# Polochon-street/bliss-rs

Measured on AMD Instinct MI355X. Metric: songs/sec (3-min 22 050 Hz f32) at 1/2/4/8 GPU; HBM GB/s vs roofline, higher is better.
Workload: dtype f32; 1 GPU; configs[1]: batch of 1024 synthetic 3969000-sample (3-min) white-noise f32 PCM buffers per GPU, full 23-feature descriptor set (FeaturesVersion 2); songs_per_gpu=1024, songs_total=1024, features=23, parallelism=single GPU

## Files before the change

bliss-rs_amd/csrc/blissgpu.hip:

```cpp
#include <math.h>
#include <stdio.h>
#include <stdlib.h>
#include <string.h>

#include <algorithm>
#include <atomic>
#include <chrono>
#include <deque>
#include <mutex>
#include <string>
#include <vector>

#include "ctx.hpp"
#include "forest.hpp"

using namespace bg;

namespace {
thread_local std::string g_last_error;

const char* const kKernelNames[K_COUNT] = {
    "fft512_kernel",     "onset_kernel",      "beat_kernel",   "stft8192_kernel", "tune_select_kernel",
    "tune_pass2_kernel", "tune_final_kernel", "chroma_kernel",     "summary_kernel", "assemble_kernel", "pairwise_kernel", "set_distance_kernel", "song_to_song_kernel", "synth_kernel", "rolloff_fix_kernel",
    "dedup_next_kernel", "dedup_walk_kernel", "knn_scan_kernel", "knn_merge_kernel",
    "forest_walk_kernel", "forest_finish_kernel"};
}

namespace bg {
int fail(int code, const char* what, const char* detail) {
    g_last_error = std::string(what) + ": " + (detail ? detail : "");
    return code;
}
}

namespace {

template <typename T>
int upload(T** dst, const std::vector<T>& h) {
    HIP_TRY(hipMalloc((void**)dst, h.size() * sizeof(T)));
    HIP_TRY(hipMemcpy(*dst, h.data(), h.size() * sizeof(T), hipMemcpyHostToDevice));
    return BLISSGPU_OK;
}

int build_tables(blissgpu_ctx* c) {
    const float PI_F = 3.14159265358979323846f;
    std::vector<float2> tw8(8192), tw5(512);
    for (int k = 0; k < 8192; k++) {
        const double a = -2.0 * M_PI * (double)k / 8192.0;
        tw8[k] = make_float2((float)cos(a), (float)sin(a));
    }
    for (int k = 0; k < 512; k++) {
        const double a = -2.0 * M_PI * (double)k / 512.0;
        tw5[k] = make_float2((float)cos(a), (float)sin(a));
    }
    std::vector<float> hann(8192), hannz(512), rwv(BT_LAGLEN), dfwv(BT_WINLEN);
    for (int n = 0; n < 8192; n++) hann[n] = 0.5f * (0.5f - 0.5f * cosf(2.0f * (float)n * PI_F / 8192.0f));
    for (int i = 0; i < 512; i++) hannz[i] = 0.5f * (0.5f * (1.0f - cosf(2.0f * PI_F * (float)i / 512.0f)));
    const float rayparam = 60.0f * (float)SAMPLE_RATE / 120.0f / (float)HOP_B;
    const float dfwvnorm = expf((logf(2.0f) / rayparam) * (float)(BT_WINLEN + 2));
    for (int i = 0; i < BT_LAGLEN; i++) {
        const float i_f = (float)(i + 1);
        rwv[i] = (i_f / (rayparam * rayparam)) * expf(-(i_f * i_f) / (2.0f * (rayparam * rayparam)));
    }
    for (int i = 0; i < BT_WINLEN; i++) dfwv[i] = expf((logf(2.0f) / rayparam) * (float)(i + 1)) / dfwvnorm;
    int rc;
    if ((rc = upload(&c->tw8192, tw8))) return rc;
    if ((rc = upload(&c->tw512, tw5))) return rc;
    if ((rc = upload(&c->hann8192, hann))) return rc;
    if ((rc = upload(&c->hannz512, hannz))) return rc;
    if ((rc = upload(&c->bt_rwv, rwv))) return rc;
    if ((rc = upload(&c->bt_dfwv, dfwv))) return rc;
    const size_t bank_elems = (size_t)(N_TUNING + 1) * BANK_ROWS * BANK_PITCH;
    HIP_TRY(hipMalloc((void**)&c->chroma_bank, bank_elems * sizeof(double)));
    launch_chroma_bank(c->chroma_bank, c->own_stream);
    HIP_TRY(hipGetLastError());
    HIP_TRY(hipStreamSynchronize(c->own_stream));
    c->tables = DeviceTables{c->tw8192, c->tw512, c->hann8192, c->hannz512, c->chroma_bank, c->bt_rwv, c->bt_dfwv};
    return BLISSGPU_OK;
}

std::mutex g_default_mu;
std::vector<int> g_default_devices;
struct DefaultSeat {
    std::mutex mu;
    blissgpu_ctx* ctx = nullptr;
    int fails = 0;
    bool permanent = false;
    std::chrono::steady_clock::time_point retry_at{};
    int rc = BLISSGPU_OK;
    std::string err;
};
std::deque<DefaultSeat> g_default_seats;
std::vector<uint64_t> g_default_batches;
bool g_default_init = false;
std::atomic<int64_t> g_single_song_timeout_ms{600000};

void default_init_locked() {
    if (g_default_init) return;
    g_default_init = true;
    if (const char* e = getenv("BLISSGPU_DEFAULT_DEVICES")) {
        for (const char* p = e; *p;) {
            char* end = nullptr;
            const long v = strtol(p, &end, 10);
            if (end == p) break;
            if (v >= 0 && v < 4096 && g_default_devices.size() < 64) g_default_devices.push_back((int)v);
            p = *end == ',' ? end + 1 : end;
            if (*end && *end != ',') break;
        }
    }
    if (g_default_devices.empty()) {
        int count = 0;
        if (hipGetDeviceCount(&count) != hipSuccess || count < 1) count = 1;
        for (int k = 0; k < count && k < 64; k++) g_default_devices.push_back(k);
    }
    g_default_seats.resize(g_default_devices.size());
    g_default_batches.assign(g_default_devices.size(), 0);
}

}

namespace bg {
int default_ctx_count() {
    std::lock_guard<std::mutex> lk(g_default_mu);
    default_init_locked();
    return (int)g_default_devices.size();
}
int default_ctx_at(int k, blissgpu_ctx** out) {
    DefaultSeat* seat = nullptr;
    int device = 0;
    {
        std::lock_guard<std::mutex> lk(g_default_mu);
        default_init_locked();
        if (k < 0 || k >= (int)g_default_devices.size()) return fail(BLISSGPU_ERR_INVALID, "default context", "no such default device");
        seat = &g_default_seats[(size_t)k];
        device = g_default_devices[(size_t)k];
    }
    std::lock_guard<std::mutex> lk(seat->mu);
    if (!seat->ctx) {
        const auto now = std::chrono::steady_clock::now();
        if (seat->fails == 0 || (!seat->permanent && now >= seat->retry_at)) {
            seat->rc = blissgpu_ctx_create(device, &seat->ctx);
            if (seat->rc) {
                seat->ctx = nullptr;
                seat->fails++;
                seat->permanent = seat->rc == BLISSGPU_ERR_NO_DEVICE || seat->rc == BLISSGPU_ERR_INVALID;
                seat->retry_at = now + std::chrono::milliseconds(std::min(5000, 100 << std::min(seat->fails - 1, 6)));
                seat->err = std::string("default context ") + std::to_string(k) + " (HIP device " + std::to_string(device) + "): " + blissgpu_last_error();
            } else {
                seat->fails = 0;
                seat->permanent = false;
            }
        }
    }
    if (!seat->ctx) return fail(seat->rc, "default context", seat->err.c_str());
    *out = seat->ctx;
    return BLISSGPU_OK;
}
void default_ctx_forget_failures() {
    std::lock_guard<std::mutex> lk(g_default_mu);
    default_init_locked();
    for (DefaultSeat& seat : g_default_seats) {
        std::lock_guard<std::mutex> sl(seat.mu);
        if (!seat.ctx) { seat.fails = 0; seat.permanent = false; seat.rc = BLISSGPU_OK; }
    }
}
namespace {
std::mutex g_live_mu;
std::vector<int> g_live_contexts;
std::mutex g_persistent_mu[64];
}
std::mutex& persistent_kernel_mutex(int device) { return g_persistent_mu[(unsigned)device % 64u]; }
void live_context_add(int device, int delta) {
    std::lock_guard<std::mutex> lk(g_live_mu);
    if (device < 0) return;
    if ((size_t)device >= g_live_contexts.size()) g_live_contexts.resize((size_t)device + 1, 0);
    g_live_contexts[(size_t)device] += delta;
}
int live_contexts(int device) {
    std::lock_guard<std::mutex> lk(g_live_mu);
    return device >= 0 && (size_t)device < g_live_contexts.size() ? g_live_contexts[(size_t)device] : 0;
}
int64_t single_song_timeout_ms() { return g_single_song_timeout_ms.load(); }
int default_ctx(blissgpu_ctx** out) { return default_ctx_at(0, out); }
void default_ctx_count_batch(int k) {
    std::lock_guard<std::mutex> lk(g_default_mu);
    if (k >= 0 && k < (int)g_default_batches.size()) g_default_batches[k]++;
}
}

extern "C" {
int blissgpu_default_device_count(void) { return default_ctx_count(); }
int blissgpu_default_ctx(int k, blissgpu_ctx** ctx) {
    if (!ctx) return fail(BLISSGPU_ERR_INVALID, "blissgpu_default_ctx", "NULL argument");
    *ctx = nullptr;
    return default_ctx_at(k, ctx);
}
int blissgpu_set_single_song_timeout_ms(int64_t ms) {
    constexpr int64_t TEN_YEARS_MS = 10LL * 365 * 24 * 3600 * 1000;
    g_single_song_timeout_ms.store(ms > 0 ? std::min(ms, TEN_YEARS_MS) : 600000);
    return BLISSGPU_OK;
}
int blissgpu_default_reset(void) {
    default_ctx_forget_failures();
    front_revive_all();
    return BLISSGPU_OK;
}
int blissgpu_default_device(int k) {
    std::lock_guard<std::mutex> lk(g_default_mu);
    default_init_locked();
    return (k >= 0 && k < (int)g_default_devices.size()) ? g_default_devices[k] : -1;
}
uint64_t blissgpu_default_device_batches(int k) {
    std::lock_guard<std::mutex> lk(g_default_mu);
    return (k >= 0 && k < (int)g_default_batches.size()) ? g_default_batches[k] : 0;
}
}

namespace {

int is_diag(const float* M, uint32_t d) {
    for (uint32_t i = 0; i < d; i++)
        for (uint32_t j = 0; j < d; j++)
            if (i != j && M[i * d + j] != 0.0f) return 0;
    return 1;
}

}

#define CTX_ENTER(c, who)                                                     \
    if (!(c)) return fail(BLISSGPU_ERR_INVALID, who, "ctx is NULL");          \
    std::lock_guard<std::recursive_mutex> ctx_lock_((c)->mu);                 \
    HIP_TRY(hipSetDevice((c)->device))

extern "C" {

const char* blissgpu_version(void) { return "blissgpu 0.3.0 (gfx950)"; }
const char* blissgpu_last_error(void) { return g_last_error.c_str(); }

const char* blissgpu_strerror(int code) {
    switch (code) {
        case BLISSGPU_OK: return "ok";
        case BLISSGPU_ERR_NO_DEVICE: return "no usable HIP device (this library has no CPU path)";
        case BLISSGPU_ERR_INVALID: return "invalid argument";
        case BLISSGPU_ERR_HIP: return "HIP runtime error";
        case BLISSGPU_ERR_NAN: return "a distance is NaN";
        case BLISSGPU_ERR_OOM: return "out of device memory";
        case BLISSGPU_ERR_RCCL: return "RCCL error";
        case BLISSGPU_ERR_TIMEOUT: return "no default context picked the call up within its deadline";
        default: return "unknown error";
    }
}

uint32_t blissgpu_feature_count(uint32_t v) { return v == BLISSGPU_FEATURES_V1 ? 20u : (v == BLISSGPU_FEATURES_V2 ? 23u : 0u); }

int blissgpu_ctx_create(int device, blissgpu_ctx** out) {
    if (!out) return fail(BLISSGPU_ERR_INVALID, "blissgpu_ctx_create", "ctx is NULL");
    int count = 0;
    hipError_t e = hipGetDeviceCount(&count);
    if (e != hipSuccess || count <= 0 || device < 0 || device >= count)
        return fail(BLISSGPU_ERR_NO_DEVICE, "hipGetDeviceCount", e != hipSuccess ? hipGetErrorString(e) : "no such device");
    HIP_TRY(hipSetDevice(device));
    blissgpu_ctx* c = new blissgpu_ctx();
    c->device = device;
    (void)hipDeviceGetAttribute(&c->n_cus, hipDeviceAttributeMultiprocessorCount, device);
    hipError_t se = hipStreamCreateWithFlags(&c->own_stream, hipStreamNonBlocking);
    if (se != hipSuccess) { delete c; return fail(BLISSGPU_ERR_HIP, "hipStreamCreate", hipGetErrorString(se)); }
    c->stream = c->own_stream;
    int prio_least = 0, prio_greatest = 0;
    (void)hipDeviceGetStreamPriorityRange(&prio_least, &prio_greatest);
    const int prio_aux = prio_greatest;
    se = hipStreamCreateWithPriority(&c->aux_stream, hipStreamNonBlocking, prio_aux);
    if (se == hipSuccess) se = hipStreamCreateWithPriority(&c->chr_stream, hipStreamNonBlocking, prio_greatest);
    if (se == hipSuccess) se = hipEventCreateWithFlags(&c->ev_interop, hipEventDisableTiming);
    if (se == hipSuccess) se = hipHostMalloc((void**)&c->h_scalar, 64, hipHostMallocDefault);
    if (se != hipSuccess) { blissgpu_ctx_destroy(c); return fail(BLISSGPU_ERR_HIP, "aux stream/events", hipGetErrorString(se)); }
    size_t free_b = 0, total_b = 0;
    if (hipMemGetInfo(&free_b, &total_b) == hipSuccess && free_b > 0)
        c->ws_limit = std::max<uint64_t>(256ull << 20, std::min<uint64_t>(64ull << 30, free_b / 3));
    else
        c->ws_limit = 16ull << 30;
    int rc = build_tables(c);
    if (rc) { blissgpu_ctx_destroy(c); return rc; }
    live_context_add(device, 1);
    c->counted_live = true;
    *out = c;
    return BLISSGPU_OK;
}

int blissgpu_ctx_destroy(blissgpu_ctx* c) {
    if (!c) return BLISSGPU_OK;
    if (c->counted_live) live_context_add(c->device, -1);
    {
        std::lock_guard<std::recursive_mutex> lk(c->mu);
        (void)hipSetDevice(c->device);
        (void)hipStreamSynchronize(c->stream);
        if (c->aux_stream) (void)hipStreamSynchronize(c->aux_stream);
        if (c->chr_stream) (void)hipStreamSynchronize(c->chr_stream);
        if (c->mask_stream) { (void)hipStreamSynchronize(c->mask_stream); (void)hipStreamDestroy(c->mask_stream); }
        for (auto& v : c->events)
            for (auto& ev : v) { (void)hipEventDestroy(ev.a); (void)hipEventDestroy(ev.b); }
        (void)hipFree(c->tw8192); (void)hipFree(c->tw512); (void)hipFree(c->hann8192); (void)hipFree(c->hannz512);
        (void)hipFree(c->bt_rwv); (void)hipFree(c->bt_dfwv); (void)hipFree(c->chroma_bank);
        scheduler_release(c);
        c->dbg_tuning.release(); c->dbg_nbpms.release(); c->dbg_chroma.release(); c->dbg_interval.release();
        c->pl_sync.release(); c->pl_keys.release(); c->pl_tmp.release(); c->pl_slots.release(); c->pl_next.release(); c->st_idx.release();
        c->st_a.release(); c->st_b.release(); c->st_m.release(); c->st_dist.release(); c->st_out.release();
        if (c->h_scalar) (void)hipHostFree(c->h_scalar);
        if (c->aux_stream) (void)hipStreamDestroy(c->aux_stream);
        if (c->chr_stream) (void)hipStreamDestroy(c->chr_stream);
        if (c->ev_interop) (void)hipEventDestroy(c->ev_interop);
        if (c->own_stream) (void)hipStreamDestroy(c->own_stream);
    }
    delete c;
    return BLISSGPU_OK;
}

int blissgpu_ctx_set_stream(blissgpu_ctx* c, void* s) {
    CTX_ENTER(c, "blissgpu_ctx_set_stream");
    (void)hipStreamSynchronize(c->stream);
    c->stream = s ? (hipStream_t)s : c->own_stream;
    return BLISSGPU_OK;
}
void* blissgpu_ctx_get_stream(blissgpu_ctx* c) { return c ? (void*)c->stream : nullptr; }

int blissgpu_ctx_wait_stream(blissgpu_ctx* c, void* producer_stream) {
    CTX_ENTER(c, "blissgpu_ctx_wait_stream");
// ... 856 lines not shown
```

bliss-rs_amd/csrc/internal.hpp:

```cpp
#pragma once
#include <hip/hip_runtime.h>
#include <stdint.h>

namespace bg {

constexpr uint32_t SAMPLE_RATE = 22050;
constexpr int W512 = 512;
constexpr int HOP_T = 128;
constexpr int HOP_B = 256;
constexpr int W8192 = 8192;
constexpr int HOP_C = 2205;
constexpr int CBINS = W8192 / 2 + 1;
constexpr int CBINS_PAD = 4128;
constexpr int BANK_PITCH = CBINS_PAD;
constexpr int BANK_ROWS = 12;
constexpr int LOUD_W = 1024;
constexpr int MIN_SAMPLES = 8192;
constexpr int N_TUNING = 100;
constexpr int PIP_LO = 57, PIP_HI = 1483;
constexpr int PIP_MAX_PER_FRAME = 714;
constexpr int CAND_BUDGET_PER_FRAME = 48;
#ifndef COARSE_SHIFT
#define COARSE_SHIFT 17
#endif
constexpr uint32_t COARSE_LOW_MASK = (1u << COARSE_SHIFT) - 1u;
constexpr int H1_BINS = 1 << (31 - COARSE_SHIFT);
constexpr int BT_WINLEN = 512, BT_STEP = 128, BT_LAGLEN = 128;
constexpr int BT_PRE_STRIDE = 264;
constexpr int F512_TILE = 512;
constexpr int CH_TILE = 64;
constexpr int STFT_TILE = 16;

struct SongDesc {
    uint64_t pcm_off;
    uint64_t n;
    uint64_t t_off;
    uint64_t b_off;
    uint64_t c_off;
    uint64_t e_off;
    uint32_t n_t;
    uint32_t n_b;
    uint32_t n_f;
    uint32_t n_c;
    uint32_t n_e;
    uint32_t n_l;
    uint32_t row;
    uint32_t ok;
};

struct RollFix {
    float* mags;
    uint32_t cap;
};
constexpr float ROLLOFF_UNPROVEN = -1.0f;

struct TuningState {
    uint32_t n_peaks;
    uint32_t b_lo, b_hi;
    uint32_t below;
    uint32_t n_cand;
    int32_t tuning_idx;
    uint32_t cand_off;
    uint32_t cand_cap;
};

struct TempoState {
    float tempo;
    uint32_t n_bpms;
};

struct DeviceTables {
    const float2* tw8192;
    const float2* tw512;
    const float* hann8192;
    const float* hannz512;
    const double* chroma_bank;
    const float* bt_rwv;
    const float* bt_dfwv;
};

enum KernelId : int {
    K_FFT512 = 0,
    K_ONSET,
    K_BEAT,
    K_STFT8192,
    K_TUNE_SELECT,
    K_TUNE_PASS2,
    K_TUNE_FINAL,
    K_CHROMA,
    K_SUMMARY,
    K_FINALIZE,
    K_PAIRWISE, K_SET_DISTANCE, K_SONG_TO_SONG,
    K_SYNTH,
    K_ROLLFIX,
    K_DEDUP_NEXT, K_DEDUP_WALK,
    K_KNN_SCAN, K_KNN_MERGE,
    K_FOREST_WALK, K_FOREST_FINISH,
    K_COUNT
};

__device__ __forceinline__ uint32_t find_segment(const uint32_t* __restrict__ prefix, uint32_t n, uint32_t x) {
    uint32_t lo = 0, hi = n;
    while (hi - lo > 1) {
        const uint32_t mid = (lo + hi) >> 1;
        if (prefix[mid] <= x) lo = mid; else hi = mid;
    }
    return lo;
}

struct Workspace {
    float *centroid, *rolloff, *flatness;
    float *flux, *thresholded;
    float* e256;
    uint32_t* zc256;
    float* spec;
    float* frame_max;
    uint32_t* h1;
    uint32_t* hist100;
    TuningState* tuning;
    uint32_t* peak_rec;
    uint32_t* peak_cnt;
    double* cand_mag;
    uint8_t* cand_pb;
    uint32_t* cand_cursor;
    uint32_t cand_cap;
    double* chroma_part;
    double* dbg_chroma;
    double* dbg_interval;
    TempoState* tempo;
    float* run_bpm;
    uint32_t* run_cnt;
    uint32_t runs_pitch;
    float* bt_pre;
    float* summary;
    RollFix* roll_fix;
    size_t roll_fix_bytes;
};

struct Batch {
    const float* pcm;
    const SongDesc* songs;
    uint32_t n_songs;
    const uint32_t* pfx_f;
    const uint32_t* pfx_c;
    const uint32_t* pfx_ct;
    const uint32_t* pfx_cw;
    uint32_t tiles_f, tiles_c, tiles_ct, tiles_cw;
    uint64_t total_b;
    uint32_t max_nb;
    uint32_t max_nt;
};

void launch_fft512(const Batch&, const Workspace&, const DeviceTables&, hipStream_t, bool rolloff_exact_all = false, bool seq_flux = false);
void launch_rolloff_fix(const Batch&, const Workspace&, uint64_t total_t, hipStream_t);
void launch_onset(const Batch&, const Workspace&, hipStream_t);
void launch_beat(const Batch&, const Workspace&, const DeviceTables&, hipStream_t);
void launch_beat_acf(const Batch&, const Workspace&, const DeviceTables&, hipStream_t);
void launch_beat_track(const Batch&, const Workspace&, const DeviceTables&, hipStream_t);
void launch_stft8192(const Batch&, const Workspace&, const DeviceTables&, hipStream_t, int shape = 0);
struct SongRange { uint32_t s0, s1, ct0, ct1, cw0, cw1; };
void launch_tune_select(const Batch&, const Workspace&, hipStream_t, const SongRange* r = nullptr);
void launch_tune_pass2(const Batch&, const Workspace&, hipStream_t, const SongRange* r = nullptr);
void launch_tune_final(const Batch&, const Workspace&, hipStream_t, const SongRange* r = nullptr);
void launch_chroma(const Batch&, const Workspace&, const DeviceTables&, hipStream_t, const SongRange* r = nullptr);
void launch_summary(const Batch&, const Workspace&, hipStream_t);
void launch_finalize(const Batch&, const Workspace&, uint32_t features_version, float* d_out, int32_t* d_status,
                     int32_t* dbg_tuning, uint32_t* dbg_nbpms, hipStream_t);
void launch_chroma_bank(double* bank, hipStream_t);
void launch_pcm_convert(const void* in, int sample_format, uint32_t channels, float* out, uint64_t frames, hipStream_t st);
struct SwrPlan;
hipError_t launch_resample(const void* in, int sample_format, uint32_t channels, uint64_t frames, const SwrPlan& plan,
                           const float* d_bank, float* out, uint64_t n_out, hipStream_t st);
void launch_pair_distance(const float* a, const float* b, uint32_t d, int metric, const float* d_M, float* out, hipStream_t st);
void launch_set_distance(const float* seeds, uint32_t n_seeds, const float* cand, uint64_t n, uint32_t d, int metric,
                         const float* M, float* dist, uint32_t* keys, uint32_t* idx, uint32_t* nan_flag, hipStream_t st);
hipError_t sort_pairs_u32(void* tmp, size_t* tmp_bytes, uint32_t* keys_in, uint32_t* keys_out, uint32_t* vals_in,
                          uint32_t* vals_out, uint32_t n, hipStream_t st, uint32_t* sync = nullptr, uint32_t max_coresident = 0);
void launch_song_to_song(const float* seeds, uint32_t n_seeds, const float* cand, uint32_t n, uint32_t d, int metric,
                         const float* M, uint32_t* order, unsigned long long* slots, uint32_t* sync, uint32_t grid,
                         hipStream_t st);
void launch_dedup_next(const float* x, uint64_t n, uint32_t d, const uint32_t* seq, uint32_t len, const uint32_t* meta,
                       int metric, const float* M, float thr, uint32_t* next, uint32_t* bad, hipStream_t st);
void launch_dedup_walk(const float* x, uint64_t n, uint32_t d, const uint32_t* seq, uint32_t len, const uint32_t* meta,
                       int metric, const float* M, float thr, const uint32_t* next, uint32_t* kept, uint64_t* n_kept,
                       uint32_t* nan_flag, uint32_t* bad, hipStream_t st);
struct KnnPlan {
    uint32_t cap;
    uint32_t qb;
    uint32_t n_split;
    uint32_t blocks_per_split;
    uint32_t grid_qb;
    uint64_t part_keys;
};
KnnPlan knn_plan(uint64_t q, uint64_t n, uint32_t k, int n_cus);
void launch_knn_scan(const float* Q, uint64_t q, const float* X, uint32_t n, uint32_t d, int metric, const float* M,
                     int m_is_diag, const uint32_t* skip, uint32_t k, const KnnPlan& p, unsigned long long* part,
                     uint32_t* nan_flag, uint32_t* bad_flag, hipStream_t st);
void launch_knn_merge(const unsigned long long* part, uint64_t q, uint32_t k, const KnnPlan& p, uint32_t* idx, float* dist,
                      hipStream_t st);
void launch_pairwise(const float* A, uint64_t n, const float* B, uint64_t m, uint32_t d, int metric, const float* M,
                     int m_is_diag, float* out, uint64_t ld_out, hipStream_t);
void launch_synth(float* pcm, const SongDesc* songs, uint32_t n_songs, const uint32_t* pfx_e, uint32_t tiles_e,
                  uint32_t first_song_index, const uint32_t* d_song_index, hipStream_t);

}
```

bliss-rs_amd/csrc/kernels_chroma.hip:

```cpp
#include <float.h>
#include <stdlib.h>

#include <type_traits>

#include "device_utils.hpp"
#include "fft_r16.hpp"
#include "internal.hpp"

namespace bg {

typedef double double4_t __attribute__((ext_vector_type(4)));

__device__ __forceinline__ double tuning_of_slot(int slot) {
    return slot >= N_TUNING ? 0.0 : (-50.0 + (100.0 * 0.01 * (double)slot)) / 100.0;
}

__global__ __launch_bounds__(256) void chroma_bank_kernel(double* __restrict__ bank) {
#pragma clang fp contract(off)
    const int slot = blockIdx.y;
    const int k = blockIdx.x * 256 + threadIdx.x;
    if (k >= BANK_PITCH) return;
    double* out = bank + (size_t)slot * BANK_ROWS * BANK_PITCH;
    if (k >= CBINS) {
        for (int r = 0; r < BANK_ROWS; r++) out[(size_t)r * BANK_PITCH + k] = 0.0;
// ... 291 lines not shown
    f2 v[16];
    if (f_first < sd.n_c) {
        load_frame(f_first, v);
        load_window();
#pragma unroll
        for (int n1 = 0; n1 < 16; n1++) v[n1] = v[n1] * win[n1];
    }
    TRACE_START();
#pragma unroll 1
    for (int fi = 0; fi < STFT_FRAMES_PER_WG; fi++) {
        const uint32_t f = f_first + (uint32_t)(STFT_GROUP * fi);
        if (f >= sd.n_c) break;
        radix16(v);
#pragma unroll
        for (int k1 = 1; k1 < 16; k1++)
            v[R16(k1)] = cmul_pk(v[R16(k1)], tw_at(hi4, k1));
        if constexpr (NARROW) {
            f2 u[16];
#pragma unroll
            for (int k1 = 0; k1 < 16; k1++) ldsf[k1 * EXN1_PITCH + t] = v[R16(k1)].x;
            __syncthreads();
#pragma unroll
            for (int m1 = 0; m1 < 16; m1++) u[m1].x = ldsf[lo4 * EXN1_PITCH + 16 * m1 + hi4];
            __syncthreads();
#pragma unroll
            for (int k1 = 0; k1 < 16; k1++) ldsf[k1 * EXN1_PITCH + t] = v[R16(k1)].y;
            __syncthreads();
#pragma unroll
            for (int m1 = 0; m1 < 16; m1++) u[m1].y = ldsf[lo4 * EXN1_PITCH + 16 * m1 + hi4];
#pragma unroll
            for (int m1 = 0; m1 < 16; m1++) v[m1] = u[m1];
        } else {
#pragma unroll
        for (int k1 = 0; k1 < 16; k1++) lds[k1 * EX1_PITCH + t] = v[R16(k1)];
        TRACE(0);
        __syncthreads();
        TRACE(1);
#pragma unroll
        for (int m1 = 0; m1 < 16; m1++) v[m1] = lds[lo4 * EX1_PITCH + 16 * m1 + hi4];
        }
        radix16(v);
        v[R16(0)] = cmul_pk(v[R16(0)], c_p2);
#pragma unroll
        for (int j1 = 1; j1 < 16; j1++) v[R16(j1)] = cmul_pk(v[R16(j1)], cmul_pk(tw_at(hi4, j1), c_p2));
        TRACE(2);
        __syncthreads();
        TRACE(3);
        if constexpr (NARROW) {
            f2 u[16];
#pragma unroll
            for (int j1 = 0; j1 < 16; j1++) ldsf[j1 * EX2_PITCH + t] = v[R16(j1)].x;
            __syncthreads();
#pragma unroll
            for (int m2 = 0; m2 < 16; m2++) u[m2].x = ldsf[hi4 * EX2_PITCH + 16 * m2 + lo4];
            __syncthreads();
#pragma unroll
            for (int j1 = 0; j1 < 16; j1++) ldsf[j1 * EX2_PITCH + t] = v[R16(j1)].y;
            __syncthreads();
#pragma unroll
            for (int m2 = 0; m2 < 16; m2++) u[m2].y = ldsf[hi4 * EX2_PITCH + 16 * m2 + lo4];
#pragma unroll
            for (int m2 = 0; m2 < 16; m2++) v[m2] = u[m2];
        } else {
#pragma unroll
        for (int j1 = 0; j1 < 16; j1++) lds[j1 * EX2_PITCH + t] = v[R16(j1)];
        TRACE(4);
        __syncthreads();
        TRACE(5);
#pragma unroll
        for (int m2 = 0; m2 < 16; m2++) v[m2] = lds[hi4 * EX2_PITCH + 16 * m2 + lo4];
        }
        radix16(v);
        TRACE(6);
        __syncthreads();
        TRACE(7);
        constexpr int ZOFF = NARROW ? 2048 : 0;
#pragma unroll
        for (int j2 = 8; j2 < 16; j2++) lds[t + 256 * j2 - ZOFF] = v[R16(j2)];
        TRACE(8);
        __syncthreads();
        TRACE(9);
        float m_lo[8], m_hi[8], m_mid = 0.0f;
        float mx = 0.0f;
#pragma unroll
        for (int j = 0; j < 8; j++) {
            const float CJ = CONST_COS32[j], SJ = CONST_SIN32[j];
            const int k = t + 256 * j;
            float sq_k, sq_m;
            const f2 w = j == 0 ? c_sp : cmul_pk_s(c_sp, mk(CJ, -SJ));
            const f2 zm = lds[(k == 0 ? 2048 : 4096 - k) - ZOFF];
            split_pair_sq(v[R16(j)], (j == 0 && t == 0) ? v[R16(0)] : zm, w, sq_k, sq_m);
            m_lo[j] = mag_from_sq(sq_k);
            m_hi[j] = mag_from_sq(sq_m);
            mx = fmaxf(mx, fmaxf(m_lo[j], m_hi[j]));
        }
        if (t == 0) {
            m_mid = mag_from_sq(split_one_sq(v[R16(8)], v[R16(8)], mk(0.0f, -1.0f)));
            mx = fmaxf(mx, m_mid);
        }
        const bool has_next = fi + 1 < STFT_FRAMES_PER_WG && f + STFT_GROUP < sd.n_c;
        if (has_next) load_frame(f + STFT_GROUP, v);
        mx = wave_max_dpp(mx);
        if constexpr (NARROW) __syncthreads();
        float* mags = reinterpret_cast<float*>(lds);
        float* mags_top = mags + MAGS_TOP_W - 4096;
#pragma unroll
        for (int j = 0; j < 8; j++) {
            mags[t + 256 * j] = m_lo[j];
            if (j == 0 && t == 0) mags_top[4096] = m_hi[0];
            else mags[4096 - (t + 256 * j)] = m_hi[j];
        }
        if (t == 0) mags[2048] = m_mid;
        if (t >= 1 && t < CBINS_PAD - 4096) mags_top[4096 + t] = 0.0f;
        {
            int slot = t >> 6;
            asm volatile("" : "+v"(slot));
            if (lane_id() == 0) red[slot] = mx;
        }
        if (t == 0) peak_count = 0;
        TRACE(10);
        __syncthreads();
        TRACE(11);
        auto store_row = [&]() {
            const __amdgpu_buffer_rsrc_t r_row = __builtin_amdgcn_make_buffer_rsrc(
                (void*)(spec + (sd.c_off + f) * (size_t)CBINS_PAD), 0, CBINS_PAD * 4, 0x00020000);
            const u32x4_t* mags4 = reinterpret_cast<const u32x4_t*>(lds);
#pragma unroll
            for (int i = 0; i < 5; i++) {
                const int q = t + 256 * i;
                if (i < 4 || q < CBINS_PAD / 4) {
                    const u32x4_t val = i < 4 ? mags4[q] : mags4[q - 1024 + MAGS_TOP_W / 4];
                    __builtin_amdgcn_raw_buffer_store_b128(val, r_row, 16u * (uint32_t)q, 0, 2);
                }
            }
        };
        store_row();
        mx = fmaxf(fmaxf(red[0], red[1]), fmaxf(red[2], red[3]));
        if (t == 0) frame_max[sd.c_off + f] = mx;
        if (!have_base) {
            if (t == 0) {
                const uint32_t top = coarse_bin((double)mx);
                lhist_base = top > (uint32_t)(LHIST_BINS * 3 / 4) ? top - (uint32_t)(LHIST_BINS * 3 / 4) : 0u;
            }
            have_base = true;
            __syncthreads();
        }
        TRACE(12);
        const uint32_t lbase = lhist_base;
        __builtin_amdgcn_s_setprio(2);
        const double ref = 0.1 * (double)mx;
        const float thr = ref_floor_f32(ref);
        {
            uint32_t hits = 0;
#pragma unroll
            for (int h = 0; h < 2; h++) {
                float sb3[3], se3[3], sa3[3];
#pragma unroll
                for (int q = 0; q < 3; q++) {
                    const int c = t + 256 * (3 * h + q);
                    sb3[q] = mags[c > 0 ? c - 1 : 0];
                    se3[q] = mags[c];
                    sa3[q] = mags[c + 1];
                }
#pragma unroll
                for (int q = 0; q < 3; q++) {
                    const int j = 3 * h + q, c = t + 256 * j;
                    const uint32_t in_range = (256 * j >= PIP_LO && 256 * j + 255 <= PIP_HI) ? 1u : (uint32_t)(c >= PIP_LO) & (uint32_t)(c <= PIP_HI);
                    const uint32_t pk = in_range & (uint32_t)(sa3[q] <= se3[q]) & (uint32_t)(sb3[q] < se3[q]) & (uint32_t)(se3[q] > thr);
                    hits |= pk << j;
                }
            }
            const uint32_t mine = (uint32_t)__popc(hits);
            const uint32_t incl = wave_scan_incl_u32_dpp(mine);
            uint32_t wbase = 0;
            if (lane_id() == 63) wbase = atomicAdd(&peak_count, incl);
            uint32_t pos = (uint32_t)__builtin_amdgcn_readlane((int)wbase, 63) + incl - mine;
#pragma unroll
            for (int j = 0; j < 6; j++)
                if ((hits >> j) & 1u) peak_list[pos++] = (uint16_t)(t + 256 * j);
            TRACE(13);
            __syncthreads();
            TRACE(14);
            const uint32_t n_peaks = peak_count;
            uint32_t* __restrict__ recs = peak_rec + (sd.c_off + f) * (size_t)PIP_MAX_PER_FRAME;
            if (t == 0) peak_cnt[sd.c_off + f] = n_peaks;
            int c_next = t < n_peaks ? (int)peak_list[t] : PIP_LO;
            for (uint32_t i = t; i < n_peaks; i += 256) {
                const int c = c_next;
                const float sb = mags[c - 1], se = mags[c], sa = mags[c + 1];
                c_next = i + 256 < n_peaks ? (int)peak_list[i + 256] : PIP_LO;
                int pb;
                const uint32_t b = peak_classify(sb, se, sa, ref, c, &pb), rel = b - lbase;
                recs[i] = peak_record(b, pb, c);
                if (rel < (uint32_t)LHIST_BINS) atomicAdd(&lhist[rel], 1u);
                else atomicAdd(&hist[b], 1u);
            }
        }
        __builtin_amdgcn_s_setprio(0);
        if (has_next) {
            load_window();
#pragma unroll
            for (int n1 = 0; n1 < 16; n1++) v[n1] = v[n1] * win[n1];
        }
        TRACE(15);
        __syncthreads();
        TRACE(16);
    }
    TRACE_FLUSH();
    if (have_base) {
        const uint32_t lbase = lhist_base;
        for (int i = t; i < LHIST_BINS; i += 256) {
            const uint32_t c = lhist[i];
            if (c) atomicAdd(&hist[lbase + i], c);
        }
    }
}

void launch_stft8192(const Batch& b, const Workspace& w, const DeviceTables& t, hipStream_t st, int shape) {
    if (b.tiles_c == 0) return;
    auto k = stft8192_kernel<false, false>;
    if (shape == 1) k = stft8192_kernel<true, true>;
    else if (shape == 2) k = stft8192_kernel<true, false>;
    else if (shape == 3) k = stft8192_kernel<false, true>;
    hipLaunchKernelGGL(k, dim3((b.tiles_c + 31u) & ~31u), dim3(256), 0, st,
                       b.pcm, b.songs, b.n_songs, b.pfx_c, t.hann8192, t.tw8192, w.spec, w.frame_max, w.h1, w.peak_rec, w.peak_cnt,
                       b.tiles_c);
}

__global__ __launch_bounds__(256) void tune_select_kernel(const SongDesc* __restrict__ songs,
                                                          const uint32_t* __restrict__ h1,
                                                          TuningState* __restrict__ tuning,
                                                          uint32_t* __restrict__ cand_cursor, uint32_t cand_pool,
                                                          uint32_t first_song) {
    __shared__ uint32_t wsum[4];
    __shared__ uint32_t s_total, s_blo, s_bhi;
    const uint32_t s = blockIdx.x + first_song;
    const int tid = threadIdx.x;
    TuningState* ts = tuning + s;
    auto no_peaks = [&]() {
        if (tid == 0) {
            ts->n_peaks = 0; ts->tuning_idx = -1; ts->n_cand = 0; ts->b_lo = 1; ts->b_hi = 0; ts->below = 0;
            ts->cand_off = 0; ts->cand_cap = 0;
        }
    };
    if (!songs[s].ok) { no_peaks(); return; }
    const uint32_t* hist = h1 + (size_t)s * H1_BINS;
    constexpr int PER = H1_BINS / 256;
    uint32_t local[PER], sum = 0;
#pragma unroll
    for (int i = 0; i < PER; i++) { local[i] = hist[tid * PER + i]; sum += local[i]; }
    const uint32_t incl = wave_scan_incl_u32(sum);
    if (lane_id() == 63) wsum[wave_id()] = incl;
    __syncthreads();
    uint32_t base = 0;
    for (int w = 0; w < wave_id(); w++) base += wsum[w];
    if (tid == 255) s_total = base + incl;
    __syncthreads();
    const uint32_t total = s_total;
    uint32_t before = base + incl - sum;
    if (total == 0) { no_peaks(); return; }
    const uint32_t r_lo = (total - 1) / 2, r_hi = total - 1 - r_lo;
    if (tid == 0) { ts->n_peaks = total; ts->n_cand = 0; ts->tuning_idx = -1; }
#pragma unroll
    for (int i = 0; i < PER; i++) {
        const uint32_t c = local[i];
        if (c) {
            if (before <= r_lo && r_lo < before + c) { ts->b_lo = tid * PER + i; ts->below = before; s_blo = tid * PER + i; }
            if (before <= r_hi && r_hi < before + c) { ts->b_hi = tid * PER + i; s_bhi = tid * PER + i; }
        }
        before += c;
    }
    __syncthreads();
    const uint32_t blo = s_blo, bhi = s_bhi;
    uint32_t mine = 0;
#pragma unroll
    for (int i = 0; i < PER; i++) {
        const uint32_t bin = tid * PER + i;
        if (bin >= blo && bin <= bhi) mine += local[i];
    }
    mine = wave_sum(mine);
    if (lane_id() == 0) wsum[wave_id()] = mine;
    __syncthreads();
    if (tid == 0) {
        const uint32_t want = wsum[0] + wsum[1] + wsum[2] + wsum[3];
        const uint32_t off = atomicAdd(cand_cursor, want);
        if (off <= cand_pool && want <= cand_pool - off) {
            ts->cand_off = off;
            ts->cand_cap = want;
        } else {
            atomicSub(cand_cursor, want);
            ts->cand_off = 0;
            ts->cand_cap = 0;
        }
    }
}

void launch_tune_select(const Batch& b, const Workspace& w, hipStream_t st, const SongRange* r) {
    const uint32_t s0 = r ? r->s0 : 0, s1 = r ? r->s1 : b.n_songs;
    if (s1 <= s0) return;
    hipLaunchKernelGGL(tune_select_kernel, dim3(s1 - s0), dim3(256), 0, st, b.songs, w.h1, w.tuning, w.cand_cursor,
                       w.cand_cap, s0);
}

constexpr int P2_SLOW_CAP = 1024;
constexpr int P2_FRAMES_PER_WAVE = CH_TILE / 4;

__global__ __launch_bounds__(256) void tune_pass2_kernel(const SongDesc* __restrict__ songs, uint32_t n_songs,
                                                         const uint32_t* __restrict__ pfx_ct,
                                                         const float* __restrict__ spec,
                                                         const float* __restrict__ frame_max,
                                                         const uint32_t* __restrict__ peak_rec,
                                                         const uint32_t* __restrict__ peak_cnt,
                                                         TuningState* __restrict__ tuning,
                                                         uint32_t* __restrict__ hist100,
                                                         double* __restrict__ cand_mag,
                                                         uint8_t* __restrict__ cand_pb, uint32_t first_tile) {
    __shared__ uint32_t hist[N_TUNING];
    __shared__ uint32_t slow_list[4][P2_SLOW_CAP];
    const uint32_t bx = blockIdx.x + first_tile;
    const uint32_t s = find_segment(pfx_ct, n_songs, bx);
    const SongDesc sd = songs[s];
    const uint32_t tile = bx - pfx_ct[s];
    const int tid = threadIdx.x, lane = lane_id(), wave = wave_id();
    TuningState* ts = tuning + s;
    const uint32_t b_lo = ts->b_lo, b_hi = ts->b_hi;
    if (ts->n_peaks == 0) return;
    const uint32_t cand_off = ts->cand_off;
    const uint32_t cand_cap = ts->cand_cap;
    const bool pooled = cand_cap != 0;
    if (tid < N_TUNING) hist[tid] = 0;
    __syncthreads();
    uint32_t n_slow = 0;

    auto flush = [&]() {
        for (uint32_t i = lane; i < n_slow; i += WAVE) {
            const uint32_t e = slow_list[wave][i];
            const int c = (int)(e & 0xFFFFu);
            const uint32_t f = tile * CH_TILE + wave + 4 * (e >> 16);
            const float* row = spec + (sd.c_off + f) * (size_t)CBINS_PAD;
            const double ref = 0.1 * (double)frame_max[sd.c_off + f];
            double mag, pitch;
            if (pip_peak_core(row[c - 1], row[c], row[c + 1], ref, c, &mag, &pitch)) {
                const uint32_t b = coarse_bin(mag);
                if (b > b_hi) {
                    atomicAdd(&hist[pitch_bin(pitch)], 1u);
                } else if (b >= b_lo) {
                    const uint32_t slot = atomicAdd(&ts->n_cand, 1u);
                    if (pooled && slot < cand_cap) {
                        cand_mag[cand_off + slot] = mag;
                        cand_pb[cand_off + slot] = (uint8_t)pitch_bin(pitch);
                    }
                }
            }
        }
        __builtin_amdgcn_wave_barrier();
        n_slow = 0;
    };
    uint32_t n_rec_next = 0;
    {
        const uint32_t f0 = tile * CH_TILE + wave;
        if (f0 < sd.n_c) n_rec_next = peak_cnt[sd.c_off + f0];
    }
    for (int i = 0; i < P2_FRAMES_PER_WAVE; i++) {
        const uint32_t f = tile * CH_TILE + wave + 4 * i;
        if (f >= sd.n_c) break;
        const uint32_t n_rec = n_rec_next < (uint32_t)PIP_MAX_PER_FRAME ? n_rec_next : (uint32_t)PIP_MAX_PER_FRAME;
        if (i + 1 < P2_FRAMES_PER_WAVE && f + 4 < sd.n_c) n_rec_next = peak_cnt[sd.c_off + f + 4];
        const uint32_t* __restrict__ recs = peak_rec + (sd.c_off + f) * (size_t)PIP_MAX_PER_FRAME;
        if (n_slow + PIP_MAX_PER_FRAME > P2_SLOW_CAP) flush();
        for (uint32_t j0 = 0; j0 < n_rec; j0 += 4 * WAVE) {
            uint32_t r4[4];
#pragma unroll
            for (int u = 0; u < 4; u++) {
                const uint32_t j = j0 + WAVE * u + lane;
                r4[u] = j < n_rec ? recs[j] : 0xFFFFFFFFu;
            }
#pragma unroll
            for (int u = 0; u < 4; u++) {
                if (j0 + WAVE * u >= n_rec) break;
                const uint32_t j = j0 + WAVE * u + lane;
                bool slow = false;
                uint32_t c = 0;
                if (j < n_rec) {
                    const uint32_t r = r4[u];
                    const uint32_t b = r >> 18, pbf = (r >> 11) & 0x7Fu;
                    c = r & 0x7FFu;
                    if (b > b_hi) {
                        if (pbf) atomicAdd(&hist[pbf - 1], 1u);
                        else slow = true;
                    } else if (b >= b_lo) {
                        slow = true;
                    }
                }
                const uint64_t mask = __ballot(slow);
                if (mask) {
                    if (slow) slow_list[wave][n_slow + (uint32_t)__popcll(mask & ((1ull << lane) - 1ull))] = ((uint32_t)i << 16) | c;
                    n_slow += (uint32_t)__popcll(mask);
                }
            }
        }
    }
    __builtin_amdgcn_wave_barrier();
    flush();
    __syncthreads();
    if (tid < N_TUNING && hist[tid]) atomicAdd(&hist100[(size_t)s * N_TUNING + tid], hist[tid]);
}

void launch_tune_pass2(const Batch& b, const Workspace& w, hipStream_t st, const SongRange* r) {
    const uint32_t t0 = r ? r->ct0 : 0, t1 = r ? r->ct1 : b.tiles_ct;
    if (t1 <= t0) return;
    hipLaunchKernelGGL(tune_pass2_kernel, dim3(t1 - t0), dim3(256), 0, st, b.songs, b.n_songs, b.pfx_ct, w.spec,
                       w.frame_max, w.peak_rec, w.peak_cnt, w.tuning, w.hist100, w.cand_mag, w.cand_pb, t0);
}

template <typename ForEach>
__device__ uint64_t block_radix_select(ForEach&& for_each, uint32_t rank, uint32_t* hist, uint32_t* s_digit, uint32_t* s_rank,
                                       uint32_t* s_wave) {
    const int tid = threadIdx.x;
    uint64_t prefix = 0, mask = 0;
    for (int shift = 56; shift >= 0; shift -= 8) {
        hist[tid] = 0;
        __syncthreads();
        for_each([&](double mag, int) {
            const uint64_t k = f64_key(mag);
            const bool in = (k & mask) == prefix;
            const uint32_t d = (uint32_t)(k >> shift) & 0xFFu;
            const uint64_t m = __ballot(in);
            if (m != 0) {
                const int first = __ffsll((unsigned long long)m) - 1;
                const uint32_t d0 = (uint32_t)__shfl((int)d, first, WAVE);
                if (__ballot(in && d == d0) == m) {
                    if (lane_id() == first) atomicAdd(&hist[d0], (uint32_t)__popcll(m));
                } else if (in) {
                    atomicAdd(&hist[d], 1u);
                }
            }
        });
        __syncthreads();
        {
            const uint32_t h = hist[tid];
            const uint32_t incl = wave_scan_incl_u32(h);
            if (lane_id() == 63) s_wave[wave_id()] = incl;
            __syncthreads();
            uint32_t below = incl - h;
            for (int w = 0; w < wave_id(); w++) below += s_wave[w];
            if (h != 0 && below <= rank && rank < below + h) {
                *s_digit = (uint32_t)tid;
                *s_rank = rank - below;
            }
        }
        __syncthreads();
        prefix |= (uint64_t)(*s_digit) << shift;
        mask |= 0xFFull << shift;
        rank = *s_rank;
        __syncthreads();
    }
    return prefix;
}

__global__ __launch_bounds__(256) void tune_final_kernel(const SongDesc* __restrict__ songs,
                                                         TuningState* __restrict__ tuning,
                                                         const uint32_t* __restrict__ hist100,
                                                         const double* __restrict__ cand_mag,
                                                         const uint8_t* __restrict__ cand_pb,
                                                         const float* __restrict__ spec,
                                                         const float* __restrict__ frame_max,
                                                         const uint32_t* __restrict__ peak_rec,
                                                         const uint32_t* __restrict__ peak_cnt, uint32_t first_song) {
    __shared__ uint32_t hist[256];
    __shared__ uint32_t s_digit, s_rank, s_cnt_le, s_wave[4];
    __shared__ unsigned long long s_min_gt;
    const uint32_t s = blockIdx.x + first_song;
    const int tid = threadIdx.x;
    TuningState* ts = tuning + s;
    const SongDesc sd = songs[s];
    if (!sd.ok || ts->n_peaks == 0) return;
    const uint32_t total = ts->n_peaks, nc = ts->n_cand;
    const uint32_t r_lo = (total - 1) / 2, r_hi = total - 1 - r_lo;
    const uint32_t k_lo = r_lo - ts->below, k_hi = r_hi - ts->below;
    const uint32_t b_lo = ts->b_lo, b_hi = ts->b_hi;
    const bool pooled = ts->cand_cap != 0 && nc == ts->cand_cap;
    const double* v = cand_mag + ts->cand_off;
    const uint8_t* pb = cand_pb + ts->cand_off;

    auto for_each = [&](auto&& fn) {
        if (pooled) {
            for (uint32_t i0 = tid; i0 < nc; i0 += 8 * 256) {
                double m8[8];
                int b8[8];
#pragma unroll
                for (int u = 0; u < 8; u++) {
                    const uint32_t i = i0 + 256u * u;
                    m8[u] = i < nc ? v[i] : 0.0;
                    b8[u] = i < nc ? (int)pb[i] : 0;
                }
#pragma unroll
                for (int u = 0; u < 8; u++)
                    if (i0 + 256u * u < nc) fn(m8[u], b8[u]);
            }
        } else {
            for (uint32_t f = 0; f < sd.n_c; f++) {
                const uint32_t n_rec_raw = peak_cnt[sd.c_off + f];
                const uint32_t n_rec = n_rec_raw < (uint32_t)PIP_MAX_PER_FRAME ? n_rec_raw : (uint32_t)PIP_MAX_PER_FRAME;
                const uint32_t* __restrict__ recs = peak_rec + (sd.c_off + f) * (size_t)PIP_MAX_PER_FRAME;
                const float* __restrict__ row = spec + (sd.c_off + f) * (size_t)CBINS_PAD;
                const double ref = 0.1 * (double)frame_max[sd.c_off + f];
                for (uint32_t j = tid; j < n_rec; j += 256) {
                    const uint32_t r = recs[j], b = r >> 18;
                    if (b < b_lo || b > b_hi) continue;
                    const int c = (int)(r & 0x7FFu);
                    double mag, pitch;
                    if (pip_peak_core(row[c - 1], row[c], row[c + 1], ref, c, &mag, &pitch)) fn(mag, pitch_bin(pitch));
                }
            }
        }
    };

    const uint64_t key_lo = block_radix_select(for_each, k_lo, hist, &s_digit, &s_rank, s_wave);
    uint64_t key_hi = key_lo;
    if (k_hi != k_lo) {
        if (tid == 0) { s_cnt_le = 0; s_min_gt = ~0ull; }
        __syncthreads();
        uint32_t cnt = 0;
        unsigned long long mn = ~0ull;
        for_each([&](double mag, int) {
            const uint64_t k = f64_key(mag);
            if (k <= key_lo) cnt++;
            else if (k < mn) mn = k;
        });
        atomicAdd(&s_cnt_le, cnt);
        atomicMin(&s_min_gt, mn);
        __syncthreads();
        if (s_cnt_le <= k_hi) key_hi = s_min_gt;
    }
    double thr;
    {
#pragma clang fp contract(off)
        const double lo = key_f64(key_lo), hi = key_f64(key_hi);
        thr = lo + (hi - lo) / 2.0;
    }
    __syncthreads();
    if (tid < N_TUNING) hist[tid] = hist100[(size_t)s * N_TUNING + tid];
    __syncthreads();
    for_each([&](double mag, int bin) {
        if (mag >= thr) atomicAdd(&hist[bin], 1u);
    });
    __syncthreads();
    if (tid == 0) {
        uint32_t best = 0;
        for (uint32_t k = 1; k < N_TUNING; k++)
            if (hist[k] > hist[best]) best = k;
        ts->tuning_idx = (int32_t)best;
    }
}

void launch_tune_final(const Batch& b, const Workspace& w, hipStream_t st, const SongRange* r) {
    const uint32_t s0 = r ? r->s0 : 0, s1 = r ? r->s1 : b.n_songs;
    if (s1 <= s0) return;
    hipLaunchKernelGGL(tune_final_kernel, dim3(s1 - s0), dim3(256), 0, st, b.songs, w.tuning, w.hist100,
                       w.cand_mag, w.cand_pb, w.spec, w.frame_max, w.peak_rec, w.peak_cnt, s0);
}

static constexpr int TMPL_LEN[10] = {2, 2, 2, 2, 2, 2, 3, 3, 3, 3};
static constexpr int TMPL_PC[10][3] = {{0, 1, 0}, {0, 2, 0}, {0, 3, 0}, {0, 4, 0}, {0, 5, 0},
                                       {0, 6, 0}, {0, 4, 7}, {0, 3, 7}, {0, 3, 6}, {0, 4, 8}};

template <int T>
__device__ __forceinline__ double interval_feature(const double (&c)[12]) {
    double acc = 0.0;
#pragma unroll
    for (int shift = 0; shift < 12; shift++) {
        const int r0 = (TMPL_PC[T][0] + shift) % 12, r1 = (TMPL_PC[T][1] + shift) % 12;
        if (TMPL_LEN[T] == 2) {
            acc += c[r0 < r1 ? r0 : r1] * c[r0 < r1 ? r1 : r0];
        } else {
            const int r2 = (TMPL_PC[T][2] + shift) % 12;
            const int lo = r0 < r1 ? (r0 < r2 ? r0 : r2) : (r1 < r2 ? r1 : r2);
            const int hi = r0 > r1 ? (r0 > r2 ? r0 : r2) : (r1 > r2 ? r1 : r2);
            const int mid = r0 + r1 + r2 - lo - hi;
            acc += (c[lo] * c[mid]) * c[hi];
        }
    }
    return acc;
}

__global__ __launch_bounds__(256) void chroma_kernel(const SongDesc* __restrict__ songs, uint32_t n_songs, const uint32_t* __restrict__ pfx_cw,
                              const uint32_t* __restrict__ pfx_ct, const float* __restrict__ spec,
                              const double* __restrict__ bank, const TuningState* __restrict__ tuning,
                              double* __restrict__ chroma_part, double* __restrict__ dbg_chroma, uint32_t first_wg);

void launch_chroma(const Batch& b, const Workspace& w, const DeviceTables& t, hipStream_t st, const SongRange* r) {
    const uint32_t g0 = r ? r->cw0 : 0, g1 = r ? r->cw1 : b.tiles_cw;
    if (g1 <= g0) return;
    hipLaunchKernelGGL(chroma_kernel, dim3(g1 - g0), dim3(256), 0, st, b.songs, b.n_songs, b.pfx_cw, b.pfx_ct, w.spec,
                       t.chroma_bank, w.tuning, w.chroma_part, w.dbg_chroma, g0);
}

#ifndef BG_PROBE_REPLACES_CHROMA_KERNEL
__global__ __launch_bounds__(256) void chroma_kernel(const SongDesc* __restrict__ songs, uint32_t n_songs,
                                                     const uint32_t* __restrict__ pfx_cw,
                                                     const uint32_t* __restrict__ pfx_ct,
                                                     const float* __restrict__ spec,
                                                     const double* __restrict__ bank,
                                                     const TuningState* __restrict__ tuning,
                                                     double* __restrict__ chroma_part,
                                                     double* __restrict__ dbg_chroma, uint32_t first_wg) {
    __shared__ double tile_c[4][4][16][13];
    const uint32_t bx = blockIdx.x + first_wg;
    const uint32_t s = find_segment(pfx_cw, n_songs, bx);
    const SongDesc sd = songs[s];
    const int lane = lane_id(), wave = wave_id();
    const uint32_t tile64 = (bx - pfx_cw[s]) * 4 + wave;
    const uint32_t n_tiles = pfx_ct[s + 1] - pfx_ct[s];
    if (tile64 >= n_tiles) return;
    const int i16 = lane & 15, g = lane >> 4;
    const int tidx = tuning[s].tuning_idx;
    const int slot = (tidx < 0) ? N_TUNING : tidx;
    const uint32_t f0 = tile64 * CH_TILE;

    const double* __restrict__ arow = bank + ((size_t)slot * BANK_ROWS + (i16 < BANK_ROWS ? i16 : BANK_ROWS - 1)) * BANK_PITCH + 8 * g;
    const float* brow[4];
#pragma unroll
    for (int q = 0; q < 4; q++) {
        uint32_t fj = f0 + 16 * q + i16;
        if (fj >= sd.n_c) fj = sd.n_c - 1;
        brow[q] = spec + (sd.c_off + fj) * (size_t)CBINS_PAD + 8 * g;
    }
    double4_t acc[4][2];
#pragma unroll
    for (int q = 0; q < 4; q++) { acc[q][0] = double4_t{0.0, 0.0, 0.0, 0.0}; acc[q][1] = double4_t{0.0, 0.0, 0.0, 0.0}; }
    struct KBlock {
        double4_t a[2];
        float4 b[2][4];
    };
    auto k_load = [&](int k0, KBlock& kb) {
#pragma unroll
        for (int u = 0; u < 2; u++) kb.a[u] = *reinterpret_cast<const double4_t*>(arow + k0 + 4 * u);
#pragma unroll
        for (int q = 0; q < 4; q++)
#pragma unroll
            for (int u = 0; u < 2; u++) kb.b[u][q] = *reinterpret_cast<const float4*>(brow[q] + k0 + 4 * u);
        __builtin_amdgcn_sched_barrier(0);
    };
    auto k_mma = [&](const KBlock& kb) {
#pragma unroll
        for (int u = 0; u < 2; u++) {
#pragma unroll
            for (int q = 0; q < 4; q++) {
                const float4 v = kb.b[u][q];
                const double b0 = (double)v.x * (double)v.x, b1 = (double)v.y * (double)v.y;
                const double b2 = (double)v.z * (double)v.z, b3 = (double)v.w * (double)v.w;
                acc[q][0] = __builtin_amdgcn_mfma_f64_16x16x4f64(kb.a[u].x, b0, acc[q][0], 0, 0, 0);
                acc[q][1] = __builtin_amdgcn_mfma_f64_16x16x4f64(kb.a[u].y, b1, acc[q][1], 0, 0, 0);
                acc[q][0] = __builtin_amdgcn_mfma_f64_16x16x4f64(kb.a[u].z, b2, acc[q][0], 0, 0, 0);
                acc[q][1] = __builtin_amdgcn_mfma_f64_16x16x4f64(kb.a[u].w, b3, acc[q][1], 0, 0, 0);
            }
        }
    };
    constexpr int KBLOCKS = CBINS_PAD / 32;
    static_assert(CBINS_PAD % 32 == 0 && BANK_PITCH == CBINS_PAD && KBLOCKS % 2 == 1, "pairs of blocks and one last block");
    KBlock k0buf, k1buf;
    k_load(0, k0buf);
#pragma unroll 1
    for (int kb = 0; kb + 2 < KBLOCKS; kb += 2) {
        k_load(32 * (kb + 1), k1buf);
        k_mma(k0buf);
        k_load(32 * (kb + 2), k0buf);
        k_mma(k1buf);
    }
    k_mma(k0buf);
#pragma unroll
    for (int q = 0; q < 4; q++) {
        const double4_t cacc = acc[q][0] + acc[q][1];
#pragma unroll
        for (int r = 0; r < 3; r++) tile_c[wave][q][i16][g + 4 * r] = cacc[r];
    }
    __builtin_amdgcn_wave_barrier();
    double feat[10];
#pragma unroll
    for (int t = 0; t < 10; t++) feat[t] = 0.0;
    if (f0 + lane < sd.n_c) {
        double c[12], sum = 0.0;
#pragma unroll
        for (int k = 0; k < 12; k++) { c[k] = tile_c[wave][lane >> 4][lane & 15][k]; sum += fabs(c[k]); }
        if (sum < DBL_MIN) sum = 1.0;
        if (dbg_chroma) {
#pragma unroll
            for (int k = 0; k < 12; k++) dbg_chroma[(sd.c_off + f0 + lane) * 12 + k] = c[k] / sum;
        }
        double esum = 0.0;
#pragma unroll
        for (int k = 0; k < 12; k++) { c[k] = exp((c[k] / sum) * 15.0); esum += fabs(c[k]); }
        if (esum < 0.0001) esum = 1.0;
#pragma unroll
        for (int k = 0; k < 12; k++) c[k] /= esum;
        feat[0] = interval_feature<0>(c); feat[1] = interval_feature<1>(c);
        feat[2] = interval_feature<2>(c); feat[3] = interval_feature<3>(c);
        feat[4] = interval_feature<4>(c); feat[5] = interval_feature<5>(c);
        feat[6] = interval_feature<6>(c); feat[7] = interval_feature<7>(c);
        feat[8] = interval_feature<8>(c); feat[9] = interval_feature<9>(c);
    }
#pragma unroll
    for (int t = 0; t < 10; t++) {
        double v = feat[t];
        const double v1 = __shfl(v, (lane & 15) + 16, WAVE), v2 = __shfl(v, (lane & 15) + 32, WAVE), v3 = __shfl(v, (lane & 15) + 48, WAVE);
        v = __shfl(v, lane & 15, WAVE);
        v = ((v + v1) + v2) + v3;
#pragma unroll
        for (int off = 8; off > 0; off >>= 1) v += __shfl_xor(v, off, WAVE);
        if (lane == 0) chroma_part[(size_t)(pfx_ct[s] + tile64) * 10 + t] = v;
    }
}

#endif

}
```

bliss-rs_amd/csrc/kernels_fft512.hip:

```cpp
#include <float.h>
#include <stdlib.h>

#include <type_traits>

#include "device_utils.hpp"
#include "fft_r16.hpp"
#include "internal.hpp"

namespace bg {

#ifndef FFT512_PAIR_SPLIT
#define FFT512_PAIR_SPLIT 1
#endif
constexpr int GROUPS_PER_WG = 16;
constexpr int FRAMES_PER_GROUP = F512_TILE / GROUPS_PER_WG;
constexpr float ROLL_GUARD = 704.0f / 16777216.0f;
constexpr int GRP_PITCH = 272;

typedef unsigned int u32x2_t __attribute__((ext_vector_type(2)));
__device__ __forceinline__ f2 buf_load_f2(__amdgpu_buffer_rsrc_t r, uint32_t voff, uint32_t soff) {
    const u32x2_t v = __builtin_amdgcn_raw_buffer_load_b64(r, voff, soff, 0);
    return mk(__uint_as_float(v.x), __uint_as_float(v.y));
}

template <int CTRL>
__device__ __forceinline__ float dpp_mov(float v) {
    return __int_as_float(__builtin_amdgcn_update_dpp(0, __float_as_int(v), CTRL, 0xF, 0xF, true));
}
template <int CTRL>
__device__ __forceinline__ int dpp_mov(int v) {
    return __builtin_amdgcn_update_dpp(0, v, CTRL, 0xF, 0xF, true);
}
constexpr int DPP_QUAD_XOR1 = 0xB1, DPP_QUAD_XOR2 = 0x4E, DPP_ROW_HALF_MIRROR = 0x141, DPP_ROW_MIRROR = 0x140;
template <typename T>
__device__ __forceinline__ T row16_sum(T v) {
    v += dpp_mov<DPP_QUAD_XOR1>(v);
    v += dpp_mov<DPP_QUAD_XOR2>(v);
    v += dpp_mov<DPP_ROW_HALF_MIRROR>(v);
    v += dpp_mov<DPP_ROW_MIRROR>(v);
    return v;
}
__device__ __forceinline__ double row16_prod(double v) {
    auto step = [](double x, auto ctrl) {
        const long long b = __double_as_longlong(x);
        const int lo = dpp_mov<decltype(ctrl)::value>((int)(b & 0xFFFFFFFFll)), hi = dpp_mov<decltype(ctrl)::value>((int)(b >> 32));
        return x * __longlong_as_double(((long long)hi << 32) | (unsigned int)lo);
    };
    v = step(v, std::integral_constant<int, DPP_QUAD_XOR1>{});
    v = step(v, std::integral_constant<int, DPP_QUAD_XOR2>{});
    v = step(v, std::integral_constant<int, DPP_ROW_HALF_MIRROR>{});
    v = step(v, std::integral_constant<int, DPP_ROW_MIRROR>{});
    return v;
}
__device__ __forceinline__ float row16_scan_incl(float v) {
    v += dpp_mov<0x111>(v);
    v += dpp_mov<0x112>(v);
    v += dpp_mov<0x114>(v);
    v += dpp_mov<0x118>(v);
    return v;
}

#define BG_DPP_STEP(OP, DST, SRC, CTRL) OP " " DST ", " SRC ", " SRC " " CTRL " row_mask:0xf bank_mask:0xf bound_ctrl:1\n\t"
__device__ __forceinline__ void row16_sum3_scan1(float in_a, float in_b, float in_c, float in_d, float& a, float& b, float& c, float& d) {
    asm("s_nop 1\n\t"
        BG_DPP_STEP("v_add_f32_dpp", "%0", "%4", "quad_perm:[1,0,3,2]") BG_DPP_STEP("v_add_f32_dpp", "%1", "%5", "quad_perm:[1,0,3,2]")
        BG_DPP_STEP("v_add_f32_dpp", "%2", "%6", "row_shr:1") BG_DPP_STEP("v_add_f32_dpp", "%3", "%7", "quad_perm:[1,0,3,2]")
        BG_DPP_STEP("v_add_f32_dpp", "%0", "%0", "quad_perm:[2,3,0,1]") BG_DPP_STEP("v_add_f32_dpp", "%1", "%1", "quad_perm:[2,3,0,1]")
        BG_DPP_STEP("v_add_f32_dpp", "%2", "%2", "row_shr:2") BG_DPP_STEP("v_add_f32_dpp", "%3", "%3", "quad_perm:[2,3,0,1]")
        BG_DPP_STEP("v_add_f32_dpp", "%0", "%0", "row_half_mirror") BG_DPP_STEP("v_add_f32_dpp", "%1", "%1", "row_half_mirror")
        BG_DPP_STEP("v_add_f32_dpp", "%2", "%2", "row_shr:4") BG_DPP_STEP("v_add_f32_dpp", "%3", "%3", "row_half_mirror")
        BG_DPP_STEP("v_add_f32_dpp", "%0", "%0", "row_mirror") BG_DPP_STEP("v_add_f32_dpp", "%1", "%1", "row_mirror")
        BG_DPP_STEP("v_add_f32_dpp", "%2", "%2", "row_shr:8") BG_DPP_STEP("v_add_f32_dpp", "%3", "%3", "row_mirror")
        : "=&v"(a), "=&v"(b), "=&v"(c), "=&v"(d)
        : "v"(in_a), "v"(in_b), "v"(in_c), "v"(in_d));
}
#define BG_DPP3(CTRL)                                                                                           \
    BG_DPP_STEP("v_add_f32_dpp", "%0", "%0", CTRL) BG_DPP_STEP("v_add_f32_dpp", "%1", "%1", CTRL) BG_DPP_STEP("v_add_u32_dpp", "%2", "%2", CTRL)
__device__ __forceinline__ void row16_sum2f_1u(float& a, float& b, uint32_t& c) {
    asm("s_nop 1\n\t" BG_DPP3("quad_perm:[1,0,3,2]") BG_DPP3("quad_perm:[2,3,0,1]") BG_DPP3("row_half_mirror") BG_DPP3("row_mirror")
        : "+v"(a), "+v"(b), "+v"(c));
}

struct FrameMags {
    float m[16];
    float nyq;
};

template <int R>
__device__ __forceinline__ f2& row(f2 (&raw)[16], int n1) { return raw[(R + n1) & 15]; }

__device__ __forceinline__ void fft512_load(__amdgpu_buffer_rsrc_t r_x, long rel_start, int l, f2 (&raw)[16]) {
    if (rel_start >= 0) {
        const uint32_t xoff = (uint32_t)((rel_start + 2 * l) * 4);
#pragma unroll
        for (int n1 = 0; n1 < 16; n1++) raw[n1] = buf_load_f2(r_x, xoff, 128u * n1);
    } else {
#pragma unroll
        for (int n1 = 0; n1 < 16; n1++) {
            const long idx = rel_start + 32 * n1 + 2 * l;
            raw[n1] = mk(0.0f, 0.0f);
            if (idx >= 0) raw[n1] = buf_load_f2(r_x, (uint32_t)(idx * 4), 0);
        }
    }
}

struct RegTables {
    f2 win[16];
    f2 tw256[16];
    f2 tw512[16];
};

template <int R>
__device__ __forceinline__ void fft512_compute(f2 (&raw)[16], int l, f2* tile, const RegTables& tabs, FrameMags& out) {
    f2 v[16];
    __builtin_amdgcn_s_setprio(0);
#pragma unroll
    for (int n1 = 0; n1 < 16; n1++) v[n1] = row<R>(raw, n1) * tabs.win[n1];
    radix16(v);
#pragma unroll
    for (int k1 = 1; k1 < 16; k1++) v[R16(k1)] = cmul_pk(v[R16(k1)], tabs.tw256[k1]);
    __builtin_amdgcn_s_setprio(2);
#pragma unroll
    for (int k1 = 0; k1 < 16; k1++) tile[k1 * 17 + l] = v[R16(k1)];
    __builtin_amdgcn_wave_barrier();
#pragma unroll
    for (int n2 = 0; n2 < 16; n2++) v[n2] = tile[l * 17 + n2];
    __builtin_amdgcn_wave_barrier();
    __builtin_amdgcn_s_setprio(0);
    radix16(v);
    __builtin_amdgcn_s_setprio(2);
#pragma unroll
    for (int k2 = 0; k2 < 16; k2++) tile[k2 * 17 + l] = v[R16(k2)];
    __builtin_amdgcn_wave_barrier();
    const f2 z0 = tile[0];
#if FFT512_PAIR_SPLIT
    {
        const f2 zk = tile[l * 17], zm = tile[(l == 0) ? 0 : 17 * (16 - l)];
        out.m[0] = mag_from_sq(split_one_sq(zk, zm, tabs.tw512[0]));
    }
    float mir[8];
#pragma unroll
    for (int e = 1; e <= 8; e++) {
        const f2 zk = tile[l * 17 + e], zm = tile[17 * (15 - l) + 16 - e];
        float sq_k, sq_m;
        split_pair_sq(zk, zm, tabs.tw512[e], sq_k, sq_m);
        out.m[e] = mag_from_sq(sq_k);
        if (e < 8) mir[e] = mag_from_sq(sq_m);
    }
#pragma unroll
    for (int e = 9; e < 16; e++) out.m[e] = dpp_mov<DPP_ROW_MIRROR>(mir[16 - e]);
#else
#pragma unroll
    for (int e = 0; e < 16; e++) {
        const f2 zk = tile[l * 17 + e];
        const int mi = (e == 0) ? ((l == 0) ? 0 : 17 * (16 - l)) : (17 * (15 - l) + 16 - e);
        const f2 zm = tile[mi];
        out.m[e] = mag_from_sq(split_one_sq(zk, zm, tabs.tw512[e]));
    }
#endif
    if (l == 0) out.m[0] = 2.0f * fabsf(z0.x + z0.y);
    out.nyq = 2.0f * fabsf(z0.x - z0.y);
    __builtin_amdgcn_wave_barrier();
}

__device__ __forceinline__ void add_lane_bit(uint32_t& acc, uint64_t mask) {
    asm("v_addc_co_u32_e64 %0, vcc, 0, %0, %1" : "+v"(acc) : "s"(mask) : "vcc");
}

__device__ __forceinline__ void stats128(const f2 r0, const f2 r1, const f2 r2, const f2 r3, const f2 before, bool song_start,
                                         float& ss, uint32_t& zc) {
    ss += ((r0.x * r0.x + r0.y * r0.y) + (r1.x * r1.x + r1.y * r1.y)) + ((r2.x * r2.x + r2.y * r2.y) + (r3.x * r3.x + r3.y * r3.y));
    constexpr uint64_t LOW = 0x0001000100010001ull;
    const uint64_t x0 = __ballot(r0.x > 0.0f), y0 = __ballot(r0.y > 0.0f), x1 = __ballot(r1.x > 0.0f), y1 = __ballot(r1.y > 0.0f);
    const uint64_t x2 = __ballot(r2.x > 0.0f), y2 = __ballot(r2.y > 0.0f), x3 = __ballot(r3.x > 0.0f), y3 = __ballot(r3.y > 0.0f);
    const uint64_t yb = __ballot(before.y > 0.0f), start = __builtin_amdgcn_ballot_w64(song_start);
    auto shifted = [&](uint64_t y, uint64_t prev_bits) { return ((y << 1) & ~LOW) | prev_bits; };
    const uint64_t p0 = (((yb >> 15) & ~start) | (x0 & start)) & LOW;
    add_lane_bit(zc, x0 ^ y0);
    add_lane_bit(zc, x0 ^ shifted(y0, p0));
    add_lane_bit(zc, x1 ^ y1);
    add_lane_bit(zc, x1 ^ shifted(y1, (y0 >> 15) & LOW));
    add_lane_bit(zc, x2 ^ y2);
    add_lane_bit(zc, x2 ^ shifted(y2, (y1 >> 15) & LOW));
    add_lane_bit(zc, x3 ^ y3);
    add_lane_bit(zc, x3 ^ shifted(y3, (y2 >> 15) & LOW));
}

template <bool ROLLOFF_EXACT_ALL, bool SEQ_FLUX>
__global__ __launch_bounds__(256, 2) void fft512_kernel(const float* __restrict__ pcm,
                                                        const SongDesc* __restrict__ songs, uint32_t n_songs,
                                                        const uint32_t* __restrict__ pfx_f,
                                                        const float* __restrict__ hannz,
                                                        const float2* __restrict__ tw512,
                                                        float* __restrict__ centroid, float* __restrict__ rolloff,
                                                        float* __restrict__ flatness, float* __restrict__ flux,
                                                        float* __restrict__ e256, uint32_t* __restrict__ zc256,
                                                        const RollFix* __restrict__ fix) {
    __shared__ f2 lds[GROUPS_PER_WG * GRP_PITCH];
    __shared__ float halo[GROUPS_PER_WG][16 * 16 + 1];
    RegTables tabs;
    {
        const int l0 = threadIdx.x & 15;
#pragma unroll
        for (int i = 0; i < 16; i++) {
            const float2 a = tw512[2 * ((i * l0) & 255)], b = tw512[16 * l0 + i];
            tabs.win[i] = mk(hannz[2 * (16 * i + l0)], hannz[2 * (16 * i + l0) + 1]);
            tabs.tw256[i] = mk(a.x, a.y);
            tabs.tw512[i] = mk(b.x, b.y);
        }
    }
    const uint32_t s = find_segment(pfx_f, n_songs, blockIdx.x);
    const SongDesc sd = songs[s];
    const uint32_t tile_idx = blockIdx.x - pfx_f[s];
    const int grp = threadIdx.x >> 4, l = threadIdx.x & 15;
    f2* tile = lds + grp * GRP_PITCH;

    const long k_begin = (long)tile_idx * F512_TILE + (long)grp * FRAMES_PER_GROUP;
    const long k_end = (k_begin + FRAMES_PER_GROUP < (long)sd.n_f) ? k_begin + FRAMES_PER_GROUP : (long)sd.n_f;

    const long tile_first = (long)tile_idx * F512_TILE * HOP_T - (W512 - HOP_T) - HOP_T;
    const long base = tile_first > 0 ? tile_first : 0;
    const uint64_t avail = (sd.n - (uint64_t)base) * 4;
    const __amdgpu_buffer_rsrc_t r_x = __builtin_amdgcn_make_buffer_rsrc(
        (void*)(pcm + sd.pcm_off + base), 0, (uint32_t)(avail < 0xFFFFFFFFull ? avail : 0xFFFFFFFFull), 0x00020000);

    FrameMags A, B;
    const bool active = k_begin < (long)sd.n_f;
    const int len = active ? (int)(k_end - k_begin) : 0;
    const long left_t = (long)sd.n_t - k_begin, left_b = (long)sd.n_b - (k_begin >> 1);
    const int lim_t = left_t < 0 ? 0 : (left_t > FRAMES_PER_GROUP ? FRAMES_PER_GROUP : (int)left_t);
    const int lim_b = left_b < 0 ? 0 : (left_b > FRAMES_PER_GROUP ? FRAMES_PER_GROUP : (int)left_b);
    const bool at_song_start = k_begin == 0;
    const uint32_t xoff0 = (uint32_t)(((k_begin + 2) * HOP_T - HOP_T - base + 2 * l) * 4);
    f2 raw[16];
    const bool share = active && grp > 0;
    if (active && k_begin >= 1 && !share) {
        fft512_load(r_x, k_begin * HOP_T - W512 - base, l, raw);
        fft512_compute<0>(raw, l, tile, tabs, A);
    } else {
#pragma unroll
        for (int e = 0; e < 16; e++) A.m[e] = 0.0f;
        A.nyq = 0.0f;
    }
    if (active) fft512_load(r_x, (k_begin + 1) * HOP_T - W512 - base, l, raw);

    float ss_acc = 0.0f;
    uint32_t zc_acc = 0;
    float st_total = 0.0f, st_wtotal = 0.0f, st_mant = 1.0f;
    int st_ints = 0;
    const float freq_per_bin = (float)SAMPLE_RATE / (float)W512;

    auto frame = [&](auto jc, int r_lane, FrameMags& cur, FrameMags& prev) {
        constexpr int J = decltype(jc)::value;
        const int r = __builtin_amdgcn_readfirstlane(r_lane);
        constexpr int R = (4 * J) & 15;
        stats128(row<R>(raw, 12), row<R>(raw, 13), row<R>(raw, 14), row<R>(raw, 15), row<R>(raw, 11), at_song_start && r == 0, ss_acc, zc_acc);
        __builtin_amdgcn_sched_barrier(0);
        fft512_compute<R>(raw, l, tile, tabs, cur);
        if (r + 1 < len) {
            const uint32_t soff = (uint32_t)r * (uint32_t)(HOP_T * 4);
#pragma unroll
            for (int n1 = 0; n1 < 4; n1++) row<R>(raw, n1) = buf_load_f2(r_x, xoff0, soff + 128u * n1);
        }
        if (J & 1) {
            float ss = ss_acc;
            uint32_t zc = zc_acc;
            const int qr = (r - 1) >> 1;
            const long q = (k_begin >> 1) + qr;
            ss_acc = 0.0f;
            zc_acc = 0;
            float f = 0.0f;
            if constexpr (SEQ_FLUX) {
#pragma unroll 1
            for (int step = 0; step < 16; step++) {
                const float carry = dpp_mov<0x111>(f);
                if (l == step) {
                    f = carry;
#pragma unroll
                    for (int e = 0; e < 16; e++) f += fmaxf(cur.m[e] - prev.m[e], 0.0f);
                }
            }
            f = __shfl(f, (threadIdx.x & 48) + 15, 64) + fmaxf(cur.nyq - prev.nyq, 0.0f);
            ss = row16_sum(ss);
            zc = (uint32_t)row16_sum((int)zc);
            } else {
#pragma unroll
            for (int i = 0; i < 8; i++) {
                const f2 d = mk(cur.m[2 * i], cur.m[2 * i + 1]) - mk(prev.m[2 * i], prev.m[2 * i + 1]);
                f += fmaxf(d.x, 0.0f);
                f += fmaxf(d.y, 0.0f);
            }
            if (l == 0) f += fmaxf(cur.nyq - prev.nyq, 0.0f);
            row16_sum2f_1u(ss, f, zc);
            }
            if (l == 0) { e256[sd.e_off + q] = ss; zc256[sd.e_off + q] = zc; }
            if (J == 1 && share && r == 1) {
#pragma unroll
                for (int e = 0; e < 16; e++) halo[grp][16 * e + l] = cur.m[e];
                if (l == 0) halo[grp][256] = cur.nyq;
            } else if (l == 0 && qr < lim_b) {
                flux[sd.b_off + q] = f;
            }
        }
        if (r < lim_t) {
            const float m15 = (l == 15) ? cur.nyq : cur.m[15];
            f2 s2 = mk(0.0f, 0.0f), e2 = mk(0.0f, 0.0f), q2 = mk(0.0f, 0.0f);
#pragma unroll
            for (int i = 0; i < 8; i++) {
                const f2 mp = mk(cur.m[2 * i], i == 7 ? m15 : cur.m[2 * i + 1]);
                s2 = s2 + mp;
                e2 = e2 + mp * mk((float)(2 * i), (float)(2 * i + 1));
                q2 = q2 + mp * mp;
            }
            auto hadd = [](f2 v) __attribute__((always_inline)) { float r; asm("v_add_f32 %0, %1, %2" : "=v"(r) : "v"(v.x), "v"(v.y)); return r; };
            const float sum = hadd(s2), sqsum = hadd(q2);
            const float wsum = (float)(16 * l) * sum + hadd(e2);
            float total, wtotal, incl, cum_total;
            row16_sum3_scan1(sum, wsum, sqsum, sqsum, total, wtotal, incl, cum_total);
            const float thr = cum_total * 0.95f;
            float d = (incl - sqsum) - thr;
            float near;
            uint32_t signs = 0;
#pragma unroll
            for (int i = 0; i < 8; i++) {
                const float m0 = cur.m[2 * i], m1 = i == 7 ? m15 : cur.m[2 * i + 1];
                const float d0 = fmaf(m0, m0, d);
                d = fmaf(m1, m1, d0);
                signs = __builtin_amdgcn_alignbit(signs, __float_as_uint(d0), 31);
                signs = __builtin_amdgcn_alignbit(signs, __float_as_uint(d), 31);
                if (i == 0) asm("v_min_f32 %0, |%1|, |%2|" : "=v"(near) : "v"(d0), "v"(d));
                else asm("v_min3_f32 %0, %0, |%1|, |%2|" : "+v"(near) : "v"(d0), "v"(d));
            }
            const bool risky = ROLLOFF_EXACT_ALL || (cum_total != 0.0f && (!(near > cum_total * ROLL_GUARD) || cum_total < 1e-30f));
            int expo = 0, zero = 0;
            double mant = 1.0;
#pragma unroll
            for (int h = 0; h < 2; h++) {
                const float c7 = h == 1 ? m15 : cur.m[7];
                const float* c8 = cur.m + 8 * h;
                double g = ((double)c8[0] * (double)c8[1]) * ((double)c8[2] * (double)c8[3]);
                g *= 3.273390607896142e150;
                g *= ((double)c8[4] * (double)c8[5]) * ((double)c8[6] * (double)c7);
                if (g == 0.0) zero = 1;
                const uint64_t bits = (uint64_t)__double_as_longlong(g);
                expo += (int)(bits >> 52);
                mant *= __longlong_as_double((long long)((bits & 0xFFFFFFFFFFFFFull) | 0x3FF0000000000000ull));
            }
            const int red = row16_sum((int)((uint32_t)__popc(signs) | ((uint32_t)zero << 9) | ((uint32_t)expo << 14)));
            const int c = red & 511, any_zero = (red >> 9) & 31, exps = (int)((uint32_t)red >> 14);
            mant = row16_prod(mant);
            const bool mine = l == (r & 15);
            const uint64_t risky_lanes = __builtin_amdgcn_ballot_w64(risky);
            const uint32_t grp_mask = (uint32_t)(risky_lanes >> (threadIdx.x & 48)) & 0xFFFFu;
            const int packed = c | (any_zero ? 1 << 9 : 0) | (cum_total == 0.0f ? 1 << 10 : 0) | (exps << 11) | (grp_mask != 0 ? 1 << 27 : 0);
            st_total = mine ? total : st_total;
            st_wtotal = mine ? wtotal : st_wtotal;
            st_ints = mine ? packed : st_ints;
            st_mant = mine ? (float)mant : st_mant;
            if (risky_lanes != 0) {
                if (grp_mask != 0) {
                    float4* dst = reinterpret_cast<float4*>(fix->mags + (size_t)(sd.t_off + (uint64_t)(k_begin + r)) * 256 + 16 * l);
                    dst[0] = make_float4(cur.m[0], cur.m[1], cur.m[2], cur.m[3]);
                    dst[1] = make_float4(cur.m[4], cur.m[5], cur.m[6], cur.m[7]);
                    dst[2] = make_float4(cur.m[8], cur.m[9], cur.m[10], cur.m[11]);
                    dst[3] = make_float4(cur.m[12], cur.m[13], cur.m[14], m15);
                }
            }
        }
    };
    auto finish16 = [&](int r16) {
        const int r = r16 + l;
        const long k = k_begin + r;
        if (r < len && r < lim_t) {
            const float cbin = (st_total == 0.0f) ? 0.0f : st_wtotal / st_total;
            const int st_c = st_ints & 511, st_exps = (st_ints >> 11) & 0xFFFF;
            const float rbin = (st_ints & (1 << 10)) ? 0.0f : (float)((st_c < 256) ? st_c + 1 : 256);
            float flat = 0.0f;
            if (!(st_ints & (1 << 9))) {
                const float geo = exp2f((log2f(st_mant) + (float)st_exps) / 256.0f - (1023.0f + 500.0f) / 8.0f);
                if (geo != 0.0f) flat = geo / (st_total / 256.0f);
            }
            centroid[sd.t_off + k] = freq_per_bin * fmaxf(cbin, 0.0f);
            rolloff[sd.t_off + k] = (st_ints & (1 << 27)) ? ROLLOFF_UNPROVEN : freq_per_bin * fmaxf(rbin, 0.0f);
            flatness[sd.t_off + k] = flat;
        }
    };

    for (int rb = 0; rb < len; rb += 4) {
        frame(std::integral_constant<int, 0>{}, rb, B, A);
        __builtin_amdgcn_sched_barrier(0);
        if (rb + 1 < len) frame(std::integral_constant<int, 1>{}, rb + 1, B, A);
        __builtin_amdgcn_sched_barrier(0);
        if (rb + 2 < len) frame(std::integral_constant<int, 2>{}, rb + 2, A, B);
        __builtin_amdgcn_sched_barrier(0);
        if (rb + 3 < len) frame(std::integral_constant<int, 3>{}, rb + 3, A, B);
        __builtin_amdgcn_sched_barrier(0);
        if ((rb & 15) == 12 || rb + 4 >= len) finish16(rb & ~15);
    }

    __syncthreads();
    if (grp + 1 < GROUPS_PER_WG && k_begin + FRAMES_PER_GROUP + 1 < (long)sd.n_f) {
        const long q = (k_begin + FRAMES_PER_GROUP) >> 1;
        float f = 0.0f;
        const float cn = halo[grp + 1][256];
        if constexpr (SEQ_FLUX) {
        float hc[16];
#pragma unroll
        for (int e = 0; e < 16; e++) hc[e] = halo[grp + 1][16 * e + l];
#pragma unroll 1
        for (int step = 0; step < 16; step++) {
            const float carry = dpp_mov<0x111>(f);
            if (l == step) {
                f = carry;
#pragma unroll
                for (int e = 0; e < 16; e++) f += fmaxf(hc[e] - A.m[e], 0.0f);
            }
        }
        f = __shfl(f, (threadIdx.x & 48) + 15, 64) + fmaxf(cn - A.nyq, 0.0f);
        } else {
#pragma unroll
        for (int e = 0; e < 16; e++) {
            const float c = halo[grp + 1][16 * e + l];
            f += fmaxf(c - A.m[e], 0.0f);
        }
        if (l == 0) f += fmaxf(cn - A.nyq, 0.0f);
        f = row16_sum(f);
        }
        if (l == 0 && q < (long)sd.n_b) flux[sd.b_off + q] = f;
    }

    if (active && k_end == (long)sd.n_f) {
        const float* __restrict__ x = pcm + sd.pcm_off;
        const uint64_t t0 = (uint64_t)sd.n_f * HOP_T;
        for (uint64_t q = t0 >> 8; q < (uint64_t)sd.n_e; q++) {
            const uint64_t lo = (q << 8) > t0 ? (q << 8) : t0;
            const uint64_t hi = ((q + 1) << 8) < sd.n ? ((q + 1) << 8) : sd.n;
            for (uint64_t i = lo + (uint64_t)l; i < hi; i += 16) {
                const float v = x[i], pv = x[i - 1];
                ss_acc += v * v;
                zc_acc += ((v > 0.0f) != (pv > 0.0f)) ? 1u : 0u;
            }
            const float ss = row16_sum(ss_acc);
            const uint32_t zc = (uint32_t)row16_sum((int)zc_acc);
            if (l == 0) { e256[sd.e_off + q] = ss; zc256[sd.e_off + q] = zc; }
            ss_acc = 0.0f;
            zc_acc = 0;
        }
    }
}

void launch_fft512(const Batch& b, const Workspace& w, const DeviceTables& t, hipStream_t st, bool rolloff_exact_all, bool seq_flux) {
    if (b.tiles_f == 0) return;
    auto k = fft512_kernel<false, false>;
    if (rolloff_exact_all && seq_flux) k = fft512_kernel<true, true>;
    else if (rolloff_exact_all) k = fft512_kernel<true, false>;
    else if (seq_flux) k = fft512_kernel<false, true>;
    hipLaunchKernelGGL(k, dim3(b.tiles_f), dim3(256), 0, st, b.pcm, b.songs, b.n_songs, b.pfx_f, t.hannz512,
                       t.tw512, w.centroid, w.rolloff, w.flatness, w.flux, w.e256, w.zc256, w.roll_fix);
}

}
```

bliss-rs_amd/csrc/scheduler.hip:

```cpp
#include <string.h>

#include <algorithm>
#include <chrono>
#include <condition_variable>
#include <numeric>

#include "coalescing_front.hpp"
#include "ctx.hpp"

using namespace bg;

namespace {

inline size_t align_up(size_t x, size_t a) { return (x + a - 1) / a * a; }

void fill_counts(SongDesc& d) {
    const uint64_t n = d.n;
    d.n_t = (uint32_t)((n - W512) / HOP_T + 1);
    d.n_b = (uint32_t)((n - W512) / HOP_B + 1);
    d.n_f = std::max(d.n_t, 2u * d.n_b);
    d.n_c = (uint32_t)ceilf((float)n / (float)HOP_C);
    d.n_e = (uint32_t)((n + 255) / 256);
    d.n_l = (uint32_t)((n + LOUD_W - 1) / LOUD_W);
}

size_t song_ws_bytes(const SongDesc& d) {
    if (!d.ok) return 256;
    size_t b = 0;
    b += (size_t)d.n_t * 12 + (size_t)d.n_b * 8 + (size_t)d.n_e * 8;
    b += (size_t)d.n_c * (CBINS_PAD * 4 + 4);
    b += (size_t)H1_BINS * 4 + N_TUNING * 4 + sizeof(TuningState) + sizeof(TempoState);
    b += (size_t)d.n_c * CAND_BUDGET_PER_FRAME * 9;
    b += (size_t)d.n_c * (PIP_MAX_PER_FRAME * 4 + 4);
    b += ((size_t)d.n_c / CH_TILE + 1) * 80;
    b += ((size_t)d.n_b / BT_STEP + 2) * (8 + BT_PRE_STRIDE * 4);
    return b + 4096;
}

struct Carver {
    uint8_t* base;
    size_t off = 0;
    template <typename T>
    T* take(size_t n) {
        off = align_up(off, 256);
        T* p = reinterpret_cast<T*>(base + off);
        off += n * sizeof(T);
        return p;
    }
};

struct ChunkTotals {
    uint64_t tot_t = 0, tot_b = 0, tot_c = 0, tot_e = 0;
    uint32_t max_nb = 0, max_nt = 0, max_runs = 1;
    uint32_t tiles_ct = 0;
    uint64_t cand_cap = 0;
};

Workspace carve(uint8_t* base, uint32_t ns, const ChunkTotals& t, size_t* bytes) {
    Carver m{base};
    Workspace w{};
    w.centroid = m.take<float>(t.tot_t); w.rolloff = m.take<float>(t.tot_t); w.flatness = m.take<float>(t.tot_t);
    w.flux = m.take<float>(t.tot_b); w.thresholded = m.take<float>(t.tot_b);
    w.e256 = m.take<float>(t.tot_e); w.zc256 = m.take<uint32_t>(t.tot_e);
    static_assert((size_t)(CBINS_PAD + PIP_MAX_PER_FRAME) * 4 * HOP_T >= (size_t)256 * 4 * HOP_C,
                  "the borrowed stretch must hold one 256-word entry per timbral frame: bytes per chroma frame x samples per "
                  "timbral frame >= bytes per entry x samples per chroma frame");
    w.spec = m.take<float>(t.tot_c * CBINS_PAD + 64);
    w.peak_rec = m.take<uint32_t>(t.tot_c * PIP_MAX_PER_FRAME);
    w.roll_fix_bytes = (size_t)(reinterpret_cast<uint8_t*>(w.peak_rec + t.tot_c * PIP_MAX_PER_FRAME) - reinterpret_cast<uint8_t*>(w.spec));
    w.frame_max = m.take<float>(t.tot_c);
    w.roll_fix = m.take<RollFix>(1);
    w.h1 = m.take<uint32_t>((size_t)ns * H1_BINS); w.hist100 = m.take<uint32_t>((size_t)ns * N_TUNING);
    w.tuning = m.take<TuningState>(ns);
    w.peak_cnt = m.take<uint32_t>(t.tot_c);
    w.cand_mag = m.take<double>(t.cand_cap); w.cand_pb = m.take<uint8_t>(t.cand_cap);
    w.cand_cursor = m.take<uint32_t>(4);
    w.cand_cap = (uint32_t)t.cand_cap;
    w.chroma_part = m.take<double>((size_t)t.tiles_ct * 10 + 16);
    w.tempo = m.take<TempoState>(ns);
    w.run_bpm = m.take<float>((size_t)ns * t.max_runs); w.run_cnt = m.take<uint32_t>((size_t)ns * t.max_runs);
    w.runs_pitch = t.max_runs;
    w.bt_pre = m.take<float>((size_t)(t.tot_b / BT_STEP + ns + 1) * BT_PRE_STRIDE);
    w.summary = m.take<float>((size_t)ns * 16);
    *bytes = m.off + 4096;
    return w;
}

int ensure_mask_stream(blissgpu_ctx* c, int cus) {
    cus = std::max(1, std::min(cus, c->n_cus));
    if (c->mask_stream && c->mask_cus == cus) return BLISSGPU_OK;
    if (c->mask_stream) { (void)hipStreamSynchronize(c->mask_stream); (void)hipStreamDestroy(c->mask_stream); c->mask_stream = nullptr; }
    std::vector<uint32_t> mask((size_t)(c->n_cus + 31) / 32, 0u);
    for (int i = 0; i < cus; i++) mask[(size_t)i / 32] |= 1u << (i % 32);
    HIP_TRY(hipExtStreamCreateWithCUMask(&c->mask_stream, (uint32_t)mask.size(), mask.data()));
    c->mask_cus = cus;
    return BLISSGPU_OK;
}

int ensure_slot_events(ChunkSlot& s) {
    if (s.ev_free) return BLISSGPU_OK;
    hipEvent_t* evs[] = {&s.ev_start, &s.ev_fork, &s.ev_stft, &s.ev_sel, &s.ev_tune, &s.ev_sum, &s.ev_chroma, &s.ev_desc, &s.ev_free, &s.ev_acf, &s.ev_beat};
    for (hipEvent_t* e : evs) HIP_TRY(hipEventCreateWithFlags(e, hipEventDisableTiming));
    for (hipEvent_t& e : s.ev_piece) HIP_TRY(hipEventCreateWithFlags(&e, hipEventDisableTiming));
    return BLISSGPU_OK;
}

int chunk_front(blissgpu_ctx* c, ChunkSlot& slot, const float* d_pcm, SongDesc* songs, uint32_t ns, bool only_chunk) {
    int rc = ensure_slot_events(slot);
    if (rc) return rc;
    std::vector<uint32_t> pfx_f(ns + 1, 0), pfx_c(ns + 1, 0), pfx_ct(ns + 1, 0), pfx_cw(ns + 1, 0);
    ChunkTotals t;
    for (uint32_t i = 0; i < ns; i++) {
        SongDesc& d = songs[i];
        d.t_off = t.tot_t; d.b_off = t.tot_b; d.c_off = t.tot_c; d.e_off = t.tot_e;
        if (d.ok) {
            t.tot_t += d.n_t; t.tot_b += d.n_b; t.tot_c += d.n_c; t.tot_e += d.n_e;
            t.max_nb = std::max(t.max_nb, d.n_b);
            t.max_nt = std::max(t.max_nt, d.n_t);
            t.max_runs = std::max(t.max_runs, d.n_b / BT_STEP + 1);
        }
        pfx_f[i + 1] = pfx_f[i] + (d.ok ? (d.n_f + F512_TILE - 1) / F512_TILE : 0);
        pfx_c[i + 1] = pfx_c[i] + (d.ok ? 4 * ((d.n_c + 4 * STFT_TILE - 1) / (4 * STFT_TILE)) : 0);
        pfx_ct[i + 1] = pfx_ct[i] + (d.ok ? (d.n_c + CH_TILE - 1) / CH_TILE : 0);
        pfx_cw[i + 1] = pfx_cw[i] + (d.ok ? (d.n_c + 4 * CH_TILE - 1) / (4 * CH_TILE) : 0);
    }
    t.tiles_ct = pfx_ct[ns];
    t.cand_cap = std::min<uint64_t>(t.tot_c * (uint64_t)c->cand_budget, 0xFFFFFF00ull) + 64;

    const size_t desc_bytes = align_up(ns * sizeof(SongDesc), 256) + 4 * align_up((ns + 1) * 4, 256) + 256;
    size_t need = 0;
    (void)carve(nullptr, ns, t, &need);
    if ((rc = slot.desc.ensure(desc_bytes))) return rc;
    if ((rc = slot.slab.ensure(need))) return rc;
    if (slot.used) HIP_TRY(hipEventSynchronize(slot.ev_desc));
    if ((rc = slot.h_desc.ensure(desc_bytes))) return rc;

    hipStream_t st = c->stream, sb = c->serial ? c->stream : c->aux_stream, sc = c->serial ? c->stream : c->chr_stream;
    const bool multi = !c->serial;
    if (slot.used && multi) HIP_TRY(hipStreamWaitEvent(st, slot.ev_free, 0));

    uint8_t* h = slot.h_desc.p;
    size_t o = 0;
    const size_t o_songs = o; memcpy(h + o, songs, ns * sizeof(SongDesc)); o = align_up(o + ns * sizeof(SongDesc), 256);
    const size_t o_f = o; memcpy(h + o, pfx_f.data(), (ns + 1) * 4); o = align_up(o + (ns + 1) * 4, 256);
    const size_t o_c = o; memcpy(h + o, pfx_c.data(), (ns + 1) * 4); o = align_up(o + (ns + 1) * 4, 256);
    const size_t o_ct = o; memcpy(h + o, pfx_ct.data(), (ns + 1) * 4); o = align_up(o + (ns + 1) * 4, 256);
    const size_t o_cw = o; memcpy(h + o, pfx_cw.data(), (ns + 1) * 4); o = align_up(o + (ns + 1) * 4, 256);
    HIP_TRY(hipMemcpyAsync(slot.desc.p, h, o, hipMemcpyHostToDevice, st));
    slot.used = true;

    Batch& b = slot.batch;
    b = Batch{};
    b.pcm = d_pcm;
    b.songs = reinterpret_cast<const SongDesc*>(slot.desc.p + o_songs);
    b.n_songs = ns;
    b.pfx_f = reinterpret_cast<const uint32_t*>(slot.desc.p + o_f);
    b.pfx_c = reinterpret_cast<const uint32_t*>(slot.desc.p + o_c);
    b.pfx_ct = reinterpret_cast<const uint32_t*>(slot.desc.p + o_ct);
    b.pfx_cw = reinterpret_cast<const uint32_t*>(slot.desc.p + o_cw);
    b.tiles_f = pfx_f[ns]; b.tiles_c = pfx_c[ns]; b.tiles_ct = pfx_ct[ns]; b.tiles_cw = pfx_cw[ns];
    b.total_b = t.tot_b; b.max_nb = t.max_nb; b.max_nt = t.max_nt;

    size_t used_bytes = 0;
    slot.ws = carve(slot.slab.p, ns, t, &used_bytes);
    slot.ws.dbg_chroma = nullptr;
    slot.ws.dbg_interval = nullptr;
    if (c->debug_chroma) {
        if ((rc = c->dbg_chroma.ensure((size_t)t.tot_c * 12 + 12))) return rc;
        if ((rc = c->dbg_interval.ensure((size_t)ns * 10))) return rc;
        slot.ws.dbg_chroma = c->dbg_chroma.p;
        slot.ws.dbg_interval = c->dbg_interval.p;
    }
    const Workspace& w = slot.ws;
    c->last_ws = w;
    c->last_songs.assign(songs, songs + ns);
    {
        RollFix rf{};
        if ((uint64_t)w.roll_fix_bytes / (256 * 4) < t.tot_t)
            return fail(BLISSGPU_ERR_INVALID, "chunk_front", "internal: the borrowed stretch cannot hold one exact-rolloff entry per timbral frame");
        rf.cap = (uint32_t)t.tot_t;
        rf.mags = w.spec;
        memcpy(h + o, &rf, sizeof(rf));
        HIP_TRY(hipMemcpyAsync(w.roll_fix, h + o, sizeof(rf), hipMemcpyHostToDevice, st));
    }
    HIP_TRY(hipEventRecord(slot.ev_desc, st));

    HIP_TRY(hipMemsetAsync(w.h1, 0, (size_t)ns * H1_BINS * 4, st));
    HIP_TRY(hipMemsetAsync(w.hist100, 0, (size_t)ns * N_TUNING * 4, st));
    HIP_TRY(hipMemsetAsync(w.cand_cursor, 0, 16, st));
    { Prof p(c, K_FFT512); launch_fft512(b, w, c->tables, st, c->rolloff_exact_all, c->flux_order); }
    { Prof p(c, K_ROLLFIX); launch_rolloff_fix(b, w, t.tot_t, st); }
    if (multi) {
        HIP_TRY(hipEventRecord(slot.ev_fork, st));
        HIP_TRY(hipStreamWaitEvent(sb, slot.ev_fork, 0));
    }
    { Prof p(c, K_ONSET, sb); launch_onset(b, w, sb); }
    { Prof p(c, K_SUMMARY, sb); launch_summary(b, w, sb); }
    slot.beat_masked = multi && c->tail_mode >= 2;
    if (slot.beat_masked) {
        if ((rc = ensure_mask_stream(c, c->tail_mode))) return rc;
        { Prof p(c, K_BEAT, sb); launch_beat_acf(b, w, c->tables, sb); }
        HIP_TRY(hipEventRecord(slot.ev_acf, sb));
        HIP_TRY(hipStreamWaitEvent(c->mask_stream, slot.ev_acf, 0));
        { Prof p(c, K_BEAT, c->mask_stream); launch_beat_track(b, w, c->tables, c->mask_stream); }
        HIP_TRY(hipEventRecord(slot.ev_beat, c->mask_stream));
    }
    const bool acf_early = multi && c->tail_mode == -2;
    if (acf_early) { Prof p(c, K_BEAT, sb); launch_beat_acf(b, w, c->tables, sb); }
    const bool beat_last = multi && c->tail_mode == -3;
    const bool beat_late = !slot.beat_masked && !beat_last && (c->tail_mode == 1 || acf_early || (c->tail_mode < 0 && only_chunk));
    if (!beat_late && !slot.beat_masked && !beat_last) { Prof p(c, K_BEAT, sb); launch_beat(b, w, c->tables, sb); }
    { Prof p(c, K_STFT8192); launch_stft8192(b, w, c->tables, st, c->stft_shape); }
    if (multi) {
        HIP_TRY(hipEventRecord(slot.ev_stft, st));
        HIP_TRY(hipStreamWaitEvent(sc, slot.ev_stft, 0));
    }
    slot.pieces = 0;
    if (multi && only_chunk && c->tail_split > 1 && ns >= 2) {
        const int want = std::min<int>(std::min<int>(c->tail_split, ChunkSlot::MAX_PIECES), (int)ns);
        uint32_t s0 = 0;
        for (int k = 0; k < want && s0 < ns; k++) {
            uint32_t s1 = s0 + 1;
            const uint64_t goal = (uint64_t)pfx_ct[ns] * (uint64_t)(k + 1) / (uint64_t)want;
            while (s1 < ns && (k == want - 1 || pfx_ct[s1] < goal)) s1++;
            slot.piece[slot.pieces++] = SongRange{s0, s1, pfx_ct[s0], pfx_ct[s1], pfx_cw[s0], pfx_cw[s1]};
            s0 = s1;
        }
        if (slot.pieces < 2) slot.pieces = 0;
    }
    if (slot.pieces) {
        for (int k = 0; k < slot.pieces; k++) {
            { Prof p(c, K_TUNE_SELECT, sc); launch_tune_select(b, w, sc, &slot.piece[k]); }
            if (k == 1 && beat_late) {
                HIP_TRY(hipEventRecord(slot.ev_sel, sc));
                HIP_TRY(hipStreamWaitEvent(sb, slot.ev_sel, 0));
                Prof p(c, K_BEAT, sb);
                if (acf_early) launch_beat_track(b, w, c->tables, sb); else launch_beat(b, w, c->tables, sb);
            }
            { Prof p(c, K_TUNE_PASS2, sc); launch_tune_pass2(b, w, sc, &slot.piece[k]); }
            { Prof p(c, K_TUNE_FINAL, sc); launch_tune_final(b, w, sc, &slot.piece[k]); }
            HIP_TRY(hipEventRecord(slot.ev_piece[k], sc));
        }
        if (beat_last) {
            HIP_TRY(hipStreamWaitEvent(sb, slot.ev_piece[slot.pieces - 1], 0));
            Prof p(c, K_BEAT, sb);
            launch_beat(b, w, c->tables, sb);
        }
        HIP_TRY(hipGetLastError());
        slot.back_pending = true;
        return BLISSGPU_OK;
    }
    { Prof p(c, K_TUNE_SELECT, sc); launch_tune_select(b, w, sc); }
    if (beat_late) {
        if (multi) {
            HIP_TRY(hipEventRecord(slot.ev_sel, sc));
            HIP_TRY(hipStreamWaitEvent(sb, slot.ev_sel, 0));
        }
        Prof p(c, K_BEAT, sb);
        if (acf_early) launch_beat_track(b, w, c->tables, sb); else launch_beat(b, w, c->tables, sb);
    }
    { Prof p(c, K_TUNE_PASS2, sc); launch_tune_pass2(b, w, sc); }
    { Prof p(c, K_TUNE_FINAL, sc); launch_tune_final(b, w, sc); }
    if (multi) HIP_TRY(hipEventRecord(slot.ev_tune, sc));
    if (beat_last) {
        HIP_TRY(hipStreamWaitEvent(sb, slot.ev_tune, 0));
        Prof p(c, K_BEAT, sb);
        launch_beat(b, w, c->tables, sb);
    }
    HIP_TRY(hipGetLastError());
    slot.back_pending = true;
    return BLISSGPU_OK;
}

int chunk_back(blissgpu_ctx* c, ChunkSlot& slot, uint32_t features_version, float* d_out, int32_t* d_status) {
    if (!slot.back_pending) return BLISSGPU_OK;
    slot.back_pending = false;
    hipStream_t st = c->stream, sb = c->serial ? c->stream : c->aux_stream;
    const bool multi = !c->serial;
    if (slot.pieces) {
        for (int k = 0; k < slot.pieces; k++) {
            HIP_TRY(hipStreamWaitEvent(st, slot.ev_piece[k], 0));
            Prof p(c, K_CHROMA);
            launch_chroma(slot.batch, slot.ws, c->tables, st, &slot.piece[k]);
        }
    } else {
        if (multi) HIP_TRY(hipStreamWaitEvent(st, slot.ev_tune, 0));
        Prof p(c, K_CHROMA);
        launch_chroma(slot.batch, slot.ws, c->tables, st);
    }
    if (multi) {
        HIP_TRY(hipEventRecord(slot.ev_chroma, st));
        HIP_TRY(hipStreamWaitEvent(sb, slot.ev_chroma, 0));
        if (slot.beat_masked) HIP_TRY(hipStreamWaitEvent(sb, slot.ev_beat, 0));
    }
    { Prof p(c, K_FINALIZE, sb); launch_finalize(slot.batch, slot.ws, features_version, d_out, d_status, c->dbg_tuning.p, c->dbg_nbpms.p, sb); }
    if (multi) HIP_TRY(hipEventRecord(slot.ev_free, sb));
    HIP_TRY(hipGetLastError());
    return BLISSGPU_OK;
}

}

namespace bg {

void scheduler_release(blissgpu_ctx* c) {
    for (ChunkSlot& s : c->slot) {
        s.slab.release(); s.desc.release(); s.h_desc.release();
        hipEvent_t evs[] = {s.ev_start, s.ev_fork, s.ev_stft, s.ev_sel, s.ev_tune, s.ev_sum, s.ev_chroma, s.ev_desc, s.ev_free, s.ev_acf, s.ev_beat};
        for (hipEvent_t e : evs)
            if (e) (void)hipEventDestroy(e);
        for (hipEvent_t e : s.ev_piece)
            if (e) (void)hipEventDestroy(e);
        s = ChunkSlot{};
    }
    HostFeed& f = c->feed;
    f.ring.reset();
    for (hipStream_t& ls : f.lane_stream)
        if (ls) { (void)hipStreamSynchronize(ls); (void)hipStreamDestroy(ls); ls = nullptr; }
    for (auto& row : f.ev_lane)
        for (hipEvent_t& ev : row)
            if (ev) { (void)hipEventDestroy(ev); ev = nullptr; }
    for (auto& kv : c->swr_banks)
        if (kv.second.d_bank) (void)hipFree(kv.second.d_bank);
    c->swr_banks.clear();
    c->swr_bytes = 0;
    for (hipStream_t& cs : f.copy_stream)
        if (cs) { (void)hipStreamSynchronize(cs); (void)hipStreamDestroy(cs); cs = nullptr; }
    f.h_rows.release();
    for (int b = 0; b < N_FEED_BUFFERS; b++) {
        f.pcm[b].release(); f.raw[b].release(); f.out[b].release();
        for (hipEvent_t& ev : f.ev_copied[b])
            if (ev) { (void)hipEventDestroy(ev); ev = nullptr; }
        if (f.ev_done[b]) (void)hipEventDestroy(f.ev_done[b]);
        f.ev_done[b] = nullptr;
    }
}

#ifndef FEED_GROUP_MIB
#define FEED_GROUP_MIB 512
#endif
#ifndef FEED_GROUP_PCM_FACTOR
#define FEED_GROUP_PCM_FACTOR 1
#endif
#ifndef STAGE_MIN_BYTES
#define STAGE_MIN_BYTES (8ull << 20)
#endif
int resample_bank(blissgpu_ctx* c, uint32_t rate, const ResampleBank** out, const char* who) {
    auto it = c->swr_banks.find(rate);
    if (it == c->swr_banks.end()) {
        ResampleBank rb;
        if (rate > MAX_SAMPLE_RATE || !swr_make_plan(rate, &rb.plan))
            return fail(BLISSGPU_ERR_INVALID, who, "sample_rate must be 1 .. 768000 Hz");
        std::vector<float> bank;
        swr_make_filter(rb.plan, bank);
        rb.bytes = bank.size() * sizeof(float);
        while (!c->swr_banks.empty() && c->swr_bytes + rb.bytes > (size_t)SWR_CACHE_BYTES) {
            auto lru = c->swr_banks.begin();
            for (auto q = c->swr_banks.begin(); q != c->swr_banks.end(); ++q)
                if (q->second.last_use < lru->second.last_use) lru = q;
            if (lru->second.d_bank) (void)hipFree(lru->second.d_bank);
            c->swr_bytes -= lru->second.bytes;
            c->swr_banks.erase(lru);
        }
        float* d = nullptr;
        hipError_t e = hipMalloc((void**)&d, rb.bytes);
        if (e != hipSuccess) { (void)hipGetLastError(); return fail(BLISSGPU_ERR_OOM, "hipMalloc(resample bank)", hipGetErrorString(e)); }
        e = hipMemcpy(d, bank.data(), rb.bytes, hipMemcpyHostToDevice);
        if (e != hipSuccess) { (void)hipFree(d); return fail(BLISSGPU_ERR_HIP, "hipMemcpy(resample bank)", hipGetErrorString(e)); }
        rb.d_bank = d;
        c->swr_bytes += rb.bytes;
        it = c->swr_banks.emplace(rate, rb).first;
    }
    it->second.last_use = ++c->swr_clock;
    *out = &it->second;
    return BLISSGPU_OK;
}

std::vector<int> parse_cpulist(const char* text) {
    std::vector<int> cpus;
    for (const char* p = text; p && *p;) {
        char* end = nullptr;
        const long a = strtol(p, &end, 10);
        if (end == p || a < 0) break;
        long b = a;
        if (*end == '-') {
            const char* q = end + 1;
            b = strtol(q, &end, 10);
            if (end == q || b < a) break;
        }
        for (long v = a; v <= b && cpus.size() < 4096; v++) cpus.push_back((int)v);
        p = *end == ',' ? end + 1 : end;
        if (*end != ',') break;
    }
    return cpus;
}

std::vector<int> device_local_cpus(int device) {
    char bus[32] = {0};
    if (hipDeviceGetPCIBusId(bus, (int)sizeof(bus), device) != hipSuccess) { (void)hipGetLastError(); return {}; }
    for (char* p = bus; *p; p++) *p = (char)tolower((unsigned char)*p);
    const std::string base = std::string("/sys/bus/pci/devices/") + bus;
    char line[4096] = {0};
    int node = -1;
    if (FILE* f = fopen((base + "/numa_node").c_str(), "r")) {
        if (fgets(line, sizeof(line), f)) node = atoi(line);
        fclose(f);
    }
    if (node < 0) return {};
    std::vector<int> cpus;
    if (FILE* f = fopen((base + "/local_cpulist").c_str(), "r")) {
        if (fgets(line, sizeof(line), f)) cpus = parse_cpulist(line);
        fclose(f);
    }
    return cpus;
}

int enqueue_decode(blissgpu_ctx* c, const void* d_in, int fmt, uint32_t channels, uint64_t frames, uint32_t rate, float* d_out,
                   uint64_t n_out, hipStream_t st, const char* who) {
    if (rate == SWR_OUT_RATE) {
        launch_pcm_convert(d_in, fmt, channels, d_out, frames, st);
        HIP_TRY(hipGetLastError());
        return BLISSGPU_OK;
    }
    const ResampleBank* rb;
    const int rc = resample_bank(c, rate, &rb, who);
    if (rc) return rc;
    HIP_TRY(launch_resample(d_in, fmt, channels, frames, rb->plan, rb->d_bank, d_out, n_out, st));
    return BLISSGPU_OK;
}

int analyze_host_songs(blissgpu_ctx* c, const FeedSong* in, uint32_t n_songs, uint32_t features_version, float* out,
                       int32_t* status, const char* who, float* d_rows) {
    const uint32_t d = blissgpu_feature_count(features_version);
    if (!d) return fail(BLISSGPU_ERR_INVALID, who, "features_version must be 1 or 2");
    if (n_songs == 0) return BLISSGPU_OK;
    std::vector<uint64_t> out_len(n_songs);
    bool any_raw = false;
    for (uint32_t i = 0; i < n_songs; i++) {
        const FeedSong& fs = in[i];
        if (fs.channels == 0 || fs.channels > 8) return fail(BLISSGPU_ERR_INVALID, who, "channels must be 1..8");
        if (fs.fmt != BLISSGPU_SAMPLE_F32 && fs.fmt != BLISSGPU_SAMPLE_S16 && fs.fmt != BLISSGPU_SAMPLE_S32)
            return fail(BLISSGPU_ERR_INVALID, who, "sample_format must be F32, S16 or S32");
        if (fs.rate == 0 || fs.rate > MAX_SAMPLE_RATE) return fail(BLISSGPU_ERR_INVALID, who, "sample_rate must be 1 .. 768000 Hz");
        if (fs.frames && !fs.p) return fail(BLISSGPU_ERR_INVALID, who, "NULL song pointer");
        if (fs.rate == SWR_OUT_RATE) out_len[i] = fs.frames;
        else {
            SwrPlan pl;
            swr_make_plan(fs.rate, &pl);
            out_len[i] = swr_out_len(pl, fs.frames);
        }
        any_raw = any_raw || !fs.direct();
    }
    std::lock_guard<std::recursive_mutex> lk(c->mu);
    HIP_TRY(hipSetDevice(c->device));
    HostFeed& f = c->feed;
    {
        uint32_t last_rate = SWR_OUT_RATE;
        for (uint32_t i = 0; i < n_songs; i++)
            if (in[i].rate != SWR_OUT_RATE && in[i].rate != last_rate && in[i].frames) {
                const ResampleBank* rb;
                const int brc = resample_bank(c, in[i].rate, &rb, who);
                if (brc) return brc;
                last_rate = in[i].rate;
            }
    }
    if (!f.copy_stream[N_COPY_STREAMS - 1]) {
        for (hipStream_t& cs : f.copy_stream)
            if (!cs) HIP_TRY(hipStreamCreateWithFlags(&cs, hipStreamNonBlocking));
        for (int b = 0; b < N_FEED_BUFFERS; b++) {
            for (hipEvent_t& ev : f.ev_copied[b])
                if (!ev) HIP_TRY(hipEventCreateWithFlags(&ev, hipEventDisableTiming));
            if (!f.ev_done[b]) HIP_TRY(hipEventCreateWithFlags(&f.ev_done[b], hipEventDisableTiming));
        }
    }
    std::vector<uint8_t> pageable(n_songs, 0);
    bool use_ring = false;
    if (f.stage_cfg.lanes > 0) {
        uint64_t pageable_bytes = 0;
        for (uint32_t i = 0; i < n_songs; i++) {
            if (!in[i].frames) continue;
            hipPointerAttribute_t at;
            const hipError_t pe = hipPointerGetAttributes(&at, in[i].p);
            if (pe != hipSuccess) (void)hipGetLastError();
            pageable[i] = pe != hipSuccess || at.type == hipMemoryTypeUnregistered;
            if (pageable[i]) pageable_bytes += in[i].frames * in[i].frame_bytes();
        }
        use_ring = pageable_bytes >= STAGE_MIN_BYTES;
    }
    if (use_ring) {
        StageConfig want = f.stage_cfg;
        want.lanes = std::min(want.lanes, MAX_STAGE_LANES);
        for (int l = 0; l < want.lanes; l++) {
            if (!f.lane_stream[l]) HIP_TRY(hipStreamCreateWithFlags(&f.lane_stream[l], hipStreamNonBlocking));
            for (int b = 0; b < N_FEED_BUFFERS; b++)
                if (!f.ev_lane[b][l]) HIP_TRY(hipEventCreateWithFlags(&f.ev_lane[b][l], hipEventDisableTiming));
        }
        if (!f.ring) f.ring.reset(new StagingRing<HipStageDev>(HipStageDev{c->device, f.lane_stream, {}}));
        if (!f.ring->running() || !(f.ring->config() == want) || f.stage_numa_known != f.stage_numa) {
            f.ring->stop();
            f.ring->dev().cpus = f.stage_numa ? device_local_cpus(c->device) : std::vector<int>{};
            f.stage_numa_known = f.stage_numa;
            std::string why;
            f.staged_bytes += f.ring->bytes_staged();
            if (!f.ring->start(want, &why)) use_ring = false;
        }
    }
    if (use_ring) f.staged_calls++;
    else std::fill(pageable.begin(), pageable.end(), 0);
    const int n_lanes = use_ring ? f.ring->config().lanes : 0;
    const size_t slab_bytes = use_ring ? f.ring->config().slab_bytes : 0;

    const uint64_t group_cap = (uint64_t)FEED_GROUP_MIB << 20;
    struct Group { uint32_t i0, n; std::vector<uint64_t> doff, dlen, roff; uint64_t total, raw_total, link_total; };
    std::vector<Group> groups;
    for (uint32_t i0 = 0; i0 < n_songs;) {
        Group g{i0, 0, {}, {}, {}, 0, 0, 0};
        uint32_t i1 = i0;
        while (i1 < n_songs) {
            const uint64_t raw = in[i1].direct() ? 0 : (in[i1].frames + 63) / 64 * 64 * in[i1].frame_bytes();
            const uint64_t pcm = (out_len[i1] + 63) / 64 * 64;
            const uint64_t link = in[i1].direct() ? 4 * pcm : raw;
            if (i1 > i0 && (g.link_total + link > group_cap || 4 * (g.total + pcm) > FEED_GROUP_PCM_FACTOR * group_cap || g.raw_total + raw > group_cap)) break;
            g.doff.push_back(g.total);
            g.dlen.push_back(out_len[i1]);
            g.roff.push_back(g.raw_total);
            g.total += pcm;
            g.raw_total += raw;
            g.link_total += link;
            i1++;
        }
        g.n = i1 - i0;
        groups.push_back(std::move(g));
        i0 = i1;
    }
    uint64_t max_total = 64, max_raw = 0, max_n = 1;
    for (const auto& g : groups) {
        max_total = std::max(max_total, g.total);
        max_raw = std::max(max_raw, g.raw_total);
        max_n = std::max<uint64_t>(max_n, g.n);
    }
    const int nbuf = (int)std::min<size_t>(groups.size(), (size_t)N_FEED_BUFFERS);
    int rc = BLISSGPU_OK;
    for (int b = 0; b < nbuf && !rc; b++) {
        rc = f.pcm[b].ensure(max_total);
        if (!rc && any_raw) rc = f.raw[b].ensure(max_raw + 256);
        if (!rc) rc = f.out[b].ensure(max_n * d);
    }
#ifdef FEED_ROWS_STAGED
    if (!rc) rc = f.h_rows.ensure((size_t)n_songs * d);
#endif
    if (rc) return rc;

    std::vector<uint64_t> ticket(groups.size(), 0);
    auto upload = [&](size_t gi) -> hipError_t {
        const Group& g = groups[gi];
        const int b = (int)(gi % nbuf);
        const bool wait_free = gi >= (size_t)nbuf;
        hipError_t ee = hipSuccess;
        for (int q = 0; q < N_COPY_STREAMS && ee == hipSuccess && wait_free; q++)
            ee = hipStreamWaitEvent(f.copy_stream[q], f.ev_done[b], 0);
        std::vector<StagePiece> pieces;
        for (uint32_t k = 0; k < g.n && ee == hipSuccess; k++) {
            const FeedSong& fs = in[g.i0 + k];
            if (!fs.frames) continue;
            uint8_t* dst = fs.direct() ? (uint8_t*)(f.pcm[b].p + g.doff[k]) : f.raw[b].p + g.roff[k];
// ... 439 lines not shown
```

Baseline: 27850 songs/sec.

## Fuse tune_final into tune_pass2 via last-block tickets; persistent tile-walk for fft512

Removes the separate tune_final kernel. Each tune_pass2 block now bumps a per-song ticket counter, and the last block for a song runs the median radix-select and the tuning histogram inline, reusing the slow_list shared memory. The fft512 kernel moves to a persistent phased tile-walk grid sized from twice the CU count, cutting block count and launch overhead. The cost is a serial per-song tail inside pass2 and an extra ticket array in the workspace.

```diff
diff --git a/bliss-rs_amd/csrc/blissgpu.hip b/bliss-rs_amd/csrc/blissgpu.hip
--- a/bliss-rs_amd/csrc/blissgpu.hip
+++ b/bliss-rs_amd/csrc/blissgpu.hip
@@ -21,7 +21,7 @@
 
 const char* const kKernelNames[K_COUNT] = {
     "fft512_kernel",     "onset_kernel",      "beat_kernel",   "stft8192_kernel", "tune_select_kernel",
-    "tune_pass2_kernel", "tune_final_kernel", "chroma_kernel",     "summary_kernel", "assemble_kernel", "pairwise_kernel", "set_distance_kernel", "song_to_song_kernel", "synth_kernel", "rolloff_fix_kernel",
+    "tune_pass2_kernel", "chroma_kernel",     "summary_kernel", "assemble_kernel", "pairwise_kernel", "set_distance_kernel", "song_to_song_kernel", "synth_kernel", "rolloff_fix_kernel",
     "dedup_next_kernel", "dedup_walk_kernel", "knn_scan_kernel", "knn_merge_kernel",
     "forest_walk_kernel", "forest_finish_kernel"};
 }
diff --git a/bliss-rs_amd/csrc/internal.hpp b/bliss-rs_amd/csrc/internal.hpp
--- a/bliss-rs_amd/csrc/internal.hpp
+++ b/bliss-rs_amd/csrc/internal.hpp
@@ -86,7 +86,6 @@
     K_STFT8192,
     K_TUNE_SELECT,
     K_TUNE_PASS2,
-    K_TUNE_FINAL,
     K_CHROMA,
     K_SUMMARY,
     K_FINALIZE,
@@ -117,6 +116,7 @@
     float* frame_max;
     uint32_t* h1;
     uint32_t* hist100;
+    uint32_t* tune_tickets;
     TuningState* tuning;
     uint32_t* peak_rec;
     uint32_t* peak_cnt;
@@ -151,7 +151,7 @@
     uint32_t max_nt;
 };
 
-void launch_fft512(const Batch&, const Workspace&, const DeviceTables&, hipStream_t, bool rolloff_exact_all = false, bool seq_flux = false);
+void launch_fft512(const Batch&, const Workspace&, const DeviceTables&, hipStream_t, uint32_t resident_wgs, bool rolloff_exact_all = false, bool seq_flux = false);
 void launch_rolloff_fix(const Batch&, const Workspace&, uint64_t total_t, hipStream_t);
 void launch_onset(const Batch&, const Workspace&, hipStream_t);
 void launch_beat(const Batch&, const Workspace&, const DeviceTables&, hipStream_t);
@@ -161,7 +161,6 @@
 struct SongRange { uint32_t s0, s1, ct0, ct1, cw0, cw1; };
 void launch_tune_select(const Batch&, const Workspace&, hipStream_t, const SongRange* r = nullptr);
 void launch_tune_pass2(const Batch&, const Workspace&, hipStream_t, const SongRange* r = nullptr);
-void launch_tune_final(const Batch&, const Workspace&, hipStream_t, const SongRange* r = nullptr);
 void launch_chroma(const Batch&, const Workspace&, const DeviceTables&, hipStream_t, const SongRange* r = nullptr);
 void launch_summary(const Batch&, const Workspace&, hipStream_t);
 void launch_finalize(const Batch&, const Workspace&, uint32_t features_version, float* d_out, int32_t* d_status,
diff --git a/bliss-rs_amd/csrc/kernels_chroma.hip b/bliss-rs_amd/csrc/kernels_chroma.hip
--- a/bliss-rs_amd/csrc/kernels_chroma.hip
+++ b/bliss-rs_amd/csrc/kernels_chroma.hip
@@ -617,6 +617,140 @@
                        w.cand_cap, s0);
 }
 
+template <typename ForEach>
+__device__ uint64_t block_radix_select(ForEach&& for_each, uint32_t rank, uint32_t* hist, uint32_t* s_digit, uint32_t* s_rank,
+                                       uint32_t* s_wave) {
+    const int tid = threadIdx.x;
+    uint64_t prefix = 0, mask = 0;
+    for (int shift = 56; shift >= 0; shift -= 8) {
+        hist[tid] = 0;
+        __syncthreads();
+        for_each([&](double mag, int) {
+            const uint64_t k = f64_key(mag);
+            const bool in = (k & mask) == prefix;
+            const uint32_t d = (uint32_t)(k >> shift) & 0xFFu;
+            const uint64_t m = __ballot(in);
+            if (m != 0) {
+                const int first = __ffsll((unsigned long long)m) - 1;
+                const uint32_t d0 = (uint32_t)__shfl((int)d, first, WAVE);
+                if (__ballot(in && d == d0) == m) {
+                    if (lane_id() == first) atomicAdd(&hist[d0], (uint32_t)__popcll(m));
+                } else if (in) {
+                    atomicAdd(&hist[d], 1u);
+                }
+            }
+        });
+        __syncthreads();
+        {
+            const uint32_t h = hist[tid];
+            const uint32_t incl = wave_scan_incl_u32(h);
+            if (lane_id() == 63) s_wave[wave_id()] = incl;
+            __syncthreads();
+            uint32_t below = incl - h;
+            for (int w = 0; w < wave_id(); w++) below += s_wave[w];
+            if (h != 0 && below <= rank && rank < below + h) {
+                *s_digit = (uint32_t)tid;
+                *s_rank = rank - below;
+            }
+        }
+        __syncthreads();
+        prefix |= (uint64_t)(*s_digit) << shift;
+        mask |= 0xFFull << shift;
+        rank = *s_rank;
+        __syncthreads();
+    }
+    return prefix;
+}
+
+__device__ void tune_final_song(const uint32_t s, const SongDesc& sd, TuningState* ts,
+                                const uint32_t* hist100, const double* cand_mag, const uint8_t* cand_pb,
+                                const float* __restrict__ spec, const float* __restrict__ frame_max,
+                                const uint32_t* __restrict__ peak_rec, const uint32_t* __restrict__ peak_cnt,
+                                uint32_t* scratch) {
+    uint32_t* const hist = scratch;
+    uint32_t* const s_wave = scratch + 256;
+    uint32_t &s_digit = scratch[260], &s_rank = scratch[261], &s_cnt_le = scratch[262];
+    unsigned long long& s_min_gt = *reinterpret_cast<unsigned long long*>(scratch + 264);
+    const int tid = threadIdx.x;
+    const uint32_t total = ts->n_peaks, nc = __hip_atomic_load(&ts->n_cand, __ATOMIC_RELAXED, __HIP_MEMORY_SCOPE_AGENT);
+    const uint32_t r_lo = (total - 1) / 2, r_hi = total - 1 - r_lo;
+    const uint32_t k_lo = r_lo - ts->below, k_hi = r_hi - ts->below;
+    const uint32_t b_lo = ts->b_lo, b_hi = ts->b_hi;
+    const bool pooled = ts->cand_cap != 0 && nc == ts->cand_cap;
+    const double* v = cand_mag + ts->cand_off;
+    const uint8_t* pb = cand_pb + ts->cand_off;
+
+    auto for_each = [&](auto&& fn) {
+        if (pooled) {
+            for (uint32_t i0 = tid; i0 < nc; i0 += 8 * 256) {
+                double m8[8];
+                int b8[8];
+#pragma unroll
+                for (int u = 0; u < 8; u++) {
+                    const uint32_t i = i0 + 256u * u;
+                    m8[u] = i < nc ? v[i] : 0.0;
+                    b8[u] = i < nc ? (int)pb[i] : 0;
+                }
+#pragma unroll
+                for (int u = 0; u < 8; u++)
+                    if (i0 + 256u * u < nc) fn(m8[u], b8[u]);
+            }
+        } else {
+            for (uint32_t f = 0; f < sd.n_c; f++) {
+                const uint32_t n_rec_raw = peak_cnt[sd.c_off + f];
+                const uint32_t n_rec = n_rec_raw < (uint32_t)PIP_MAX_PER_FRAME ? n_rec_raw : (uint32_t)PIP_MAX_PER_FRAME;
+                const uint32_t* __restrict__ recs = peak_rec + (sd.c_off + f) * (size_t)PIP_MAX_PER_FRAME;
+                const float* __restrict__ row = spec + (sd.c_off + f) * (size_t)CBINS_PAD;
+                const double ref = 0.1 * (double)frame_max[sd.c_off + f];
+                for (uint32_t j = tid; j < n_rec; j += 256) {
+                    const uint32_t r = recs[j], b = r >> 18;
+                    if (b < b_lo || b > b_hi) continue;
+                    const int c = (int)(r & 0x7FFu);
+                    double mag, pitch;
+                    if (pip_peak_core(row[c - 1], row[c], row[c + 1], ref, c, &mag, &pitch)) fn(mag, pitch_bin(pitch));
+                }
+            }
+        }
+    };
+
+    const uint64_t key_lo = block_radix_select(for_each, k_lo, hist, &s_digit, &s_rank, s_wave);
+    uint64_t key_hi = key_lo;
+    if (k_hi != k_lo) {
+        if (tid == 0) { s_cnt_le = 0; s_min_gt = ~0ull; }
+        __syncthreads();
+        uint32_t cnt = 0;
+        unsigned long long mn = ~0ull;
+        for_each([&](double mag, int) {
+            const uint64_t k = f64_key(mag);
+            if (k <= key_lo) cnt++;
+            else if (k < mn) mn = k;
+        });
+        atomicAdd(&s_cnt_le, cnt);
+        atomicMin(&s_min_gt, mn);
+        __syncthreads();
+        if (s_cnt_le <= k_hi) key_hi = s_min_gt;
+    }
+    double thr;
+    {
+#pragma clang fp contract(off)
+        const double lo = key_f64(key_lo), hi = key_f64(key_hi);
+        thr = lo + (hi - lo) / 2.0;
+    }
+    __syncthreads();
+    if (tid < N_TUNING) hist[tid] = hist100[(size_t)s * N_TUNING + tid];
+    __syncthreads();
+    for_each([&](double mag, int bin) {
+        if (mag >= thr) atomicAdd(&hist[bin], 1u);
+    });
+    __syncthreads();
+    if (tid == 0) {
+        uint32_t best = 0;
+        for (uint32_t k = 1; k < N_TUNING; k++)
+            if (hist[k] > hist[best]) best = k;
+        ts->tuning_idx = (int32_t)best;
+    }
+}
+
 constexpr int P2_SLOW_CAP = 1024;
 constexpr int P2_FRAMES_PER_WAVE = CH_TILE / 4;
 
@@ -628,10 +762,11 @@
                                                          const uint32_t* __restrict__ peak_cnt,
                                                          TuningState* __restrict__ tuning,
                                                          uint32_t* __restrict__ hist100,
-                                                         double* __restrict__ cand_mag,
-                                                         uint8_t* __restrict__ cand_pb, uint32_t first_tile) {
+                                                         double* cand_mag, uint8_t* cand_pb,
+                                                         uint32_t* __restrict__ tickets, uint32_t first_tile) {
     __shared__ uint32_t hist[N_TUNING];
-    __shared__ uint32_t slow_list[4][P2_SLOW_CAP];
+    __shared__ __attribute__((aligned(16))) uint32_t slow_list[4][P2_SLOW_CAP];
+    __shared__ uint32_t s_ticket;
     const uint32_t bx = blockIdx.x + first_tile;
     const uint32_t s = find_segment(pfx_ct, n_songs, bx);
     const SongDesc sd = songs[s];
@@ -719,161 +854,20 @@
     flush();
     __syncthreads();
     if (tid < N_TUNING && hist[tid]) atomicAdd(&hist100[(size_t)s * N_TUNING + tid], hist[tid]);
+    __threadfence();
+    __syncthreads();
+    if (tid == 0) s_ticket = atomicAdd(&tickets[s], 1u);
+    __syncthreads();
+    if (s_ticket + 1 != pfx_ct[s + 1] - pfx_ct[s]) return;
+    __threadfence();
+    tune_final_song(s, sd, ts, hist100, cand_mag, cand_pb, spec, frame_max, peak_rec, peak_cnt, &slow_list[0][0]);
 }
 
 void launch_tune_pass2(const Batch& b, const Workspace& w, hipStream_t st, const SongRange* r) {
     const uint32_t t0 = r ? r->ct0 : 0, t1 = r ? r->ct1 : b.tiles_ct;
     if (t1 <= t0) return;
     hipLaunchKernelGGL(tune_pass2_kernel, dim3(t1 - t0), dim3(256), 0, st, b.songs, b.n_songs, b.pfx_ct, w.spec,
-                       w.frame_max, w.peak_rec, w.peak_cnt, w.tuning, w.hist100, w.cand_mag, w.cand_pb, t0);
-}
-
-template <typename ForEach>
-__device__ uint64_t block_radix_select(ForEach&& for_each, uint32_t rank, uint32_t* hist, uint32_t* s_digit, uint32_t* s_rank,
-                                       uint32_t* s_wave) {
-    const int tid = threadIdx.x;
-    uint64_t prefix = 0, mask = 0;
-    for (int shift = 56; shift >= 0; shift -= 8) {
-        hist[tid] = 0;
-        __syncthreads();
-        for_each([&](double mag, int) {
-            const uint64_t k = f64_key(mag);
-            const bool in = (k & mask) == prefix;
-            const uint32_t d = (uint32_t)(k >> shift) & 0xFFu;
-            const uint64_t m = __ballot(in);
-            if (m != 0) {
-                const int first = __ffsll((unsigned long long)m) - 1;
-                const uint32_t d0 = (uint32_t)__shfl((int)d, first, WAVE);
-                if (__ballot(in && d == d0) == m) {
-                    if (lane_id() == first) atomicAdd(&hist[d0], (uint32_t)__popcll(m));
-                } else if (in) {
-                    atomicAdd(&hist[d], 1u);
-                }
-            }
-        });
-        __syncthreads();
-        {
-            const uint32_t h = hist[tid];
-            const uint32_t incl = wave_scan_incl_u32(h);
-            if (lane_id() == 63) s_wave[wave_id()] = incl;
-            __syncthreads();
-            uint32_t below = incl - h;
-            for (int w = 0; w < wave_id(); w++) below += s_wave[w];
-            if (h != 0 && below <= rank && rank < below + h) {
-                *s_digit = (uint32_t)tid;
-                *s_rank = rank - below;
-            }
-        }
-        __syncthreads();
-        prefix |= (uint64_t)(*s_digit) << shift;
-        mask |= 0xFFull << shift;
-        rank = *s_rank;
-        __syncthreads();
-    }
-    return prefix;
-}
-
-__global__ __launch_bounds__(256) void tune_final_kernel(const SongDesc* __restrict__ songs,
-                                                         TuningState* __restrict__ tuning,
-                                                         const uint32_t* __restrict__ hist100,
-                                                         const double* __restrict__ cand_mag,
-                                                         const uint8_t* __restrict__ cand_pb,
-                                                         const float* __restrict__ spec,
-                                                         const float* __restrict__ frame_max,
-                                                         const uint32_t* __restrict__ peak_rec,
-                                                         const uint32_t* __restrict__ peak_cnt, uint32_t first_song) {
-    __shared__ uint32_t hist[256];
-    __shared__ uint32_t s_digit, s_rank, s_cnt_le, s_wave[4];
-    __shared__ unsigned long long s_min_gt;
-    const uint32_t s = blockIdx.x + first_song;
-    const int tid = threadIdx.x;
-    TuningState* ts = tuning + s;
-    const SongDesc sd = songs[s];
-    if (!sd.ok || ts->n_peaks == 0) return;
-    const uint32_t total = ts->n_peaks, nc = ts->n_cand;
-    const uint32_t r_lo = (total - 1) / 2, r_hi = total - 1 - r_lo;
-    const uint32_t k_lo = r_lo - ts->below, k_hi = r_hi - ts->below;
-    const uint32_t b_lo = ts->b_lo, b_hi = ts->b_hi;
-    const bool pooled = ts->cand_cap != 0 && nc == ts->cand_cap;
-    const double* v = cand_mag + ts->cand_off;
-    const uint8_t* pb = cand_pb + ts->cand_off;
-
-    auto for_each = [&](auto&& fn) {
-        if (pooled) {
-            for (uint32_t i0 = tid; i0 < nc; i0 += 8 * 256) {
-                double m8[8];
-                int b8[8];
-#pragma unroll
-                for (int u = 0; u < 8; u++) {
-                    const uint32_t i = i0 + 256u * u;
-                    m8[u] = i < nc ? v[i] : 0.0;
-                    b8[u] = i < nc ? (int)pb[i] : 0;
-                }
-#pragma unroll
-                for (int u = 0; u < 8; u++)
-                    if (i0 + 256u * u < nc) fn(m8[u], b8[u]);
-            }
-        } else {
-            for (uint32_t f = 0; f < sd.n_c; f++) {
-                const uint32_t n_rec_raw = peak_cnt[sd.c_off + f];
-                const uint32_t n_rec = n_rec_raw < (uint32_t)PIP_MAX_PER_FRAME ? n_rec_raw : (uint32_t)PIP_MAX_PER_FRAME;
-                const uint32_t* __restrict__ recs = peak_rec + (sd.c_off + f) * (size_t)PIP_MAX_PER_FRAME;
-                const float* __restrict__ row = spec + (sd.c_off + f) * (size_t)CBINS_PAD;
-                const double ref = 0.1 * (double)frame_max[sd.c_off + f];
-                for (uint32_t j = tid; j < n_rec; j += 256) {
-                    const uint32_t r = recs[j], b = r >> 18;
-                    if (b < b_lo || b > b_hi) continue;
-                    const int c = (int)(r & 0x7FFu);
-                    double mag, pitch;
-                    if (pip_peak_core(row[c - 1], row[c], row[c + 1], ref, c, &mag, &pitch)) fn(mag, pitch_bin(pitch));
-                }
-            }
-        }
-    };
-
-    const uint64_t key_lo = block_radix_select(for_each, k_lo, hist, &s_digit, &s_rank, s_wave);
-    uint64_t key_hi = key_lo;
-    if (k_hi != k_lo) {
-        if (tid == 0) { s_cnt_le = 0; s_min_gt = ~0ull; }
-        __syncthreads();
-        uint32_t cnt = 0;
-        unsigned long long mn = ~0ull;
-        for_each([&](double mag, int) {
-            const uint64_t k = f64_key(mag);
-            if (k <= key_lo) cnt++;
-            else if (k < mn) mn = k;
-        });
-        atomicAdd(&s_cnt_le, cnt);
-        atomicMin(&s_min_gt, mn);
-        __syncthreads();
-        if (s_cnt_le <= k_hi) key_hi = s_min_gt;
-    }
-    double thr;
-    {
-#pragma clang fp contract(off)
-        const double lo = key_f64(key_lo), hi = key_f64(key_hi);
-        thr = lo + (hi - lo) / 2.0;
-    }
-    __syncthreads();
-    if (tid < N_TUNING) hist[tid] = hist100[(size_t)s * N_TUNING + tid];
-    __syncthreads();
-    for_each([&](double mag, int bin) {
-        if (mag >= thr) atomicAdd(&hist[bin], 1u);
-    });
-    __syncthreads();
-    if (tid == 0) {
-        uint32_t best = 0;
-        for (uint32_t k = 1; k < N_TUNING; k++)
-            if (hist[k] > hist[best]) best = k;
-        ts->tuning_idx = (int32_t)best;
-    }
-}
-
-void launch_tune_final(const Batch& b, const Workspace& w, hipStream_t st, const SongRange* r) {
-    const uint32_t s0 = r ? r->s0 : 0, s1 = r ? r->s1 : b.n_songs;
-    if (s1 <= s0) return;
-    hipLaunchKernelGGL(tune_final_kernel, dim3(s1 - s0), dim3(256), 0, st, b.songs, w.tuning, w.hist100,
-                       w.cand_mag, w.cand_pb, w.spec, w.frame_max, w.peak_rec, w.peak_cnt, s0);
+                       w.frame_max, w.peak_rec, w.peak_cnt, w.tuning, w.hist100, w.cand_mag, w.cand_pb, w.tune_tickets, t0);
 }
 
 static constexpr int TMPL_LEN[10] = {2, 2, 2, 2, 2, 2, 3, 3, 3, 3};
diff --git a/bliss-rs_amd/csrc/kernels_fft512.hip b/bliss-rs_amd/csrc/kernels_fft512.hip
--- a/bliss-rs_amd/csrc/kernels_fft512.hip
+++ b/bliss-rs_amd/csrc/kernels_fft512.hip
@@ -6,6 +6,7 @@
 #include "device_utils.hpp"
 #include "fft_r16.hpp"
 #include "internal.hpp"
+#include "tile_walk.hpp"
 
 namespace bg {
 
@@ -195,9 +196,9 @@
                                                         float* __restrict__ centroid, float* __restrict__ rolloff,
                                                         float* __restrict__ flatness, float* __restrict__ flux,
                                                         float* __restrict__ e256, uint32_t* __restrict__ zc256,
-                                                        const RollFix* __restrict__ fix) {
+                                                        const RollFix* __restrict__ fix, const WalkPlan plan) {
     __shared__ f2 lds[GROUPS_PER_WG * GRP_PITCH];
-    __shared__ float halo[GROUPS_PER_WG][16 * 16 + 1];
+    __shared__ float halo2[2][GROUPS_PER_WG][16 * 16 + 1];
     RegTables tabs;
     {
         const int l0 = threadIdx.x & 15;
@@ -209,254 +210,261 @@
             tabs.tw512[i] = mk(b.x, b.y);
         }
     }
-    const uint32_t s = find_segment(pfx_f, n_songs, blockIdx.x);
-    const SongDesc sd = songs[s];
-    const uint32_t tile_idx = blockIdx.x - pfx_f[s];
     const int grp = threadIdx.x >> 4, l = threadIdx.x & 15;
     f2* tile = lds + grp * GRP_PITCH;
-
-    const long k_begin = (long)tile_idx * F512_TILE + (long)grp * FRAMES_PER_GROUP;
-    const long k_end = (k_begin + FRAMES_PER_GROUP < (long)sd.n_f) ? k_begin + FRAMES_PER_GROUP : (long)sd.n_f;
-
-    const long tile_first = (long)tile_idx * F512_TILE * HOP_T - (W512 - HOP_T) - HOP_T;
-    const long base = tile_first > 0 ? tile_first : 0;
-    const uint64_t avail = (sd.n - (uint64_t)base) * 4;
-    const __amdgpu_buffer_rsrc_t r_x = __builtin_amdgcn_make_buffer_rsrc(
-        (void*)(pcm + sd.pcm_off + base), 0, (uint32_t)(avail < 0xFFFFFFFFull ? avail : 0xFFFFFFFFull), 0x00020000);
-
-    FrameMags A, B;
-    const bool active = k_begin < (long)sd.n_f;
-    const int len = active ? (int)(k_end - k_begin) : 0;
-    const long left_t = (long)sd.n_t - k_begin, left_b = (long)sd.n_b - (k_begin >> 1);
-    const int lim_t = left_t < 0 ? 0 : (left_t > FRAMES_PER_GROUP ? FRAMES_PER_GROUP : (int)left_t);
-    const int lim_b = left_b < 0 ? 0 : (left_b > FRAMES_PER_GROUP ? FRAMES_PER_GROUP : (int)left_b);
-    const bool at_song_start = k_begin == 0;
-    const uint32_t xoff0 = (uint32_t)(((k_begin + 2) * HOP_T - HOP_T - base + 2 * l) * 4);
-    f2 raw[16];
-    const bool share = active && grp > 0;
-    if (active && k_begin >= 1 && !share) {
-        fft512_load(r_x, k_begin * HOP_T - W512 - base, l, raw);
-        fft512_compute<0>(raw, l, tile, tabs, A);
-    } else {
-#pragma unroll
-        for (int e = 0; e < 16; e++) A.m[e] = 0.0f;
-        A.nyq = 0.0f;
-    }
-    if (active) fft512_load(r_x, (k_begin + 1) * HOP_T - W512 - base, l, raw);
-
-    float ss_acc = 0.0f;
-    uint32_t zc_acc = 0;
-    float st_total = 0.0f, st_wtotal = 0.0f, st_mant = 1.0f;
-    int st_ints = 0;
     const float freq_per_bin = (float)SAMPLE_RATE / (float)W512;
-
-    auto frame = [&](auto jc, int r_lane, FrameMags& cur, FrameMags& prev) {
-        constexpr int J = decltype(jc)::value;
-        const int r = __builtin_amdgcn_readfirstlane(r_lane);
-        constexpr int R = (4 * J) & 15;
-        stats128(row<R>(raw, 12), row<R>(raw, 13), row<R>(raw, 14), row<R>(raw, 15), row<R>(raw, 11), at_song_start && r == 0, ss_acc, zc_acc);
-        __builtin_amdgcn_sched_barrier(0);
-        fft512_compute<R>(raw, l, tile, tabs, cur);
-        if (r + 1 < len) {
-            const uint32_t soff = (uint32_t)r * (uint32_t)(HOP_T * 4);
-#pragma unroll
-            for (int n1 = 0; n1 < 4; n1++) row<R>(raw, n1) = buf_load_f2(r_x, xoff0, soff + 128u * n1);
-        }
-        if (J & 1) {
-            float ss = ss_acc;
-            uint32_t zc = zc_acc;
-            const int qr = (r - 1) >> 1;
-            const long q = (k_begin >> 1) + qr;
-            ss_acc = 0.0f;
-            zc_acc = 0;
+    uint32_t w_first, w_stride, w_end;
+    walk_enter(plan, blockIdx.x, &w_first, &w_stride, &w_end);
+#pragma unroll 1
+    for (uint32_t step = 0, wt = w_first; wt < w_end; step++, wt += w_stride) {
+        float (*halo)[16 * 16 + 1] = halo2[step & 1];
+        uint32_t tile_idx;
+        const uint32_t s = walk_locate(pfx_f, n_songs, wt, &tile_idx);
+        const SongDesc sd = songs[s];
+
+        const long k_begin = (long)tile_idx * F512_TILE + (long)grp * FRAMES_PER_GROUP;
+        const long k_end = (k_begin + FRAMES_PER_GROUP < (long)sd.n_f) ? k_begin + FRAMES_PER_GROUP : (long)sd.n_f;
+
+        const long tile_first = (long)tile_idx * F512_TILE * HOP_T - (W512 - HOP_T) - HOP_T;
+        const long base = tile_first > 0 ? tile_first : 0;
+        const uint64_t avail = (sd.n - (uint64_t)base) * 4;
+        const __amdgpu_buffer_rsrc_t r_x = __builtin_amdgcn_make_buffer_rsrc(
+            (void*)(pcm + sd.pcm_off + base), 0, (uint32_t)(avail < 0xFFFFFFFFull ? avail : 0xFFFFFFFFull), 0x00020000);
+
+        FrameMags A, B;
+        const bool active = k_begin < (long)sd.n_f;
+        const int len = active ? (int)(k_end - k_begin) : 0;
+        const long left_t = (long)sd.n_t - k_begin, left_b = (long)sd.n_b - (k_begin >> 1);
+        const int lim_t = left_t < 0 ? 0 : (left_t > FRAMES_PER_GROUP ? FRAMES_PER_GROUP : (int)left_t);
+        const int lim_b = left_b < 0 ? 0 : (left_b > FRAMES_PER_GROUP ? FRAMES_PER_GROUP : (int)left_b);
+        const bool at_song_start = k_begin == 0;
+        const uint32_t xoff0 = (uint32_t)(((k_begin + 2) * HOP_T - HOP_T - base + 2 * l) * 4);
+        f2 raw[16];
+        const bool share = active && grp > 0;
+        if (active && k_begin >= 1 && !share) {
+            fft512_load(r_x, k_begin * HOP_T - W512 - base, l, raw);
+            fft512_compute<0>(raw, l, tile, tabs, A);
+        } else {
+#pragma unroll
+            for (int e = 0; e < 16; e++) A.m[e] = 0.0f;
+            A.nyq = 0.0f;
+        }
+        if (active) fft512_load(r_x, (k_begin + 1) * HOP_T - W512 - base, l, raw);
+
+        float ss_acc = 0.0f;
+        uint32_t zc_acc = 0;
+        float st_total = 0.0f, st_wtotal = 0.0f, st_mant = 1.0f;
+        int st_ints = 0;
+
+        auto frame = [&](auto jc, int r_lane, FrameMags& cur, FrameMags& prev) {
+            constexpr int J = decltype(jc)::value;
+            const int r = __builtin_amdgcn_readfirstlane(r_lane);
+            constexpr int R = (4 * J) & 15;
+            stats128(row<R>(raw, 12), row<R>(raw, 13), row<R>(raw, 14), row<R>(raw, 15), row<R>(raw, 11), at_song_start && r == 0, ss_acc, zc_acc);
+            __builtin_amdgcn_sched_barrier(0);
+            fft512_compute<R>(raw, l, tile, tabs, cur);
+            if (r + 1 < len) {
+                const uint32_t soff = (uint32_t)r * (uint32_t)(HOP_T * 4);
+#pragma unroll
+                for (int n1 = 0; n1 < 4; n1++) row<R>(raw, n1) = buf_load_f2(r_x, xoff0, soff + 128u * n1);
+            }
+            if (J & 1) {
+                float ss = ss_acc;
+                uint32_t zc = zc_acc;
+                const int qr = (r - 1) >> 1;
+                const long q = (k_begin >> 1) + qr;
+                ss_acc = 0.0f;
+                zc_acc = 0;
+                float f = 0.0f;
+                if constexpr (SEQ_FLUX) {
+#pragma unroll 1
+                for (int step = 0; step < 16; step++) {
+                    const float carry = dpp_mov<0x111>(f);
+                    if (l == step) {
+                        f = carry;
+#pragma unroll
+                        for (int e = 0; e < 16; e++) f += fmaxf(cur.m[e] - prev.m[e], 0.0f);
+                    }
+                }
+                f = __shfl(f, (threadIdx.x & 48) + 15, 64) + fmaxf(cur.nyq - prev.nyq, 0.0f);
+                ss = row16_sum(ss);
+                zc = (uint32_t)row16_sum((int)zc);
+                } else {
+#pragma unroll
+                for (int i = 0; i < 8; i++) {
+                    const f2 d = mk(cur.m[2 * i], cur.m[2 * i + 1]) - mk(prev.m[2 * i], prev.m[2 * i + 1]);
+                    f += fmaxf(d.x, 0.0f);
+                    f += fmaxf(d.y, 0.0f);
+                }
+                if (l == 0) f += fmaxf(cur.nyq - prev.nyq, 0.0f);
+                row16_sum2f_1u(ss, f, zc);
+                }
+                if (l == 0) { e256[sd.e_off + q] = ss; zc256[sd.e_off + q] = zc; }
+                if (J == 1 && share && r == 1) {
+#pragma unroll
+                    for (int e = 0; e < 16; e++) halo[grp][16 * e + l] = cur.m[e];
+                    if (l == 0) halo[grp][256] = cur.nyq;
+                } else if (l == 0 && qr < lim_b) {
+                    flux[sd.b_off + q] = f;
+                }
+            }
+            if (r < lim_t) {
+                const float m15 = (l == 15) ? cur.nyq : cur.m[15];
+                f2 s2 = mk(0.0f, 0.0f), e2 = mk(0.0f, 0.0f), q2 = mk(0.0f, 0.0f);
+#pragma unroll
+                for (int i = 0; i < 8; i++) {
+                    const f2 mp = mk(cur.m[2 * i], i == 7 ? m15 : cur.m[2 * i + 1]);
+                    s2 = s2 + mp;
+                    e2 = e2 + mp * mk((float)(2 * i), (float)(2 * i + 1));
+                    q2 = q2 + mp * mp;
+                }
+                auto hadd = [](f2 v) __attribute__((always_inline)) { float r; asm("v_add_f32 %0, %1, %2" : "=v"(r) : "v"(v.x), "v"(v.y)); return r; };
+                const float sum = hadd(s2), sqsum = hadd(q2);
+                const float wsum = (float)(16 * l) * sum + hadd(e2);
+                float total, wtotal, incl, cum_total;
+                row16_sum3_scan1(sum, wsum, sqsum, sqsum, total, wtotal, incl, cum_total);
+                const float thr = cum_total * 0.95f;
+                float d = (incl - sqsum) - thr;
+                float near;
+                uint32_t signs = 0;
+#pragma unroll
+                for (int i = 0; i < 8; i++) {
+                    const float m0 = cur.m[2 * i], m1 = i == 7 ? m15 : cur.m[2 * i + 1];
+                    const float d0 = fmaf(m0, m0, d);
+                    d = fmaf(m1, m1, d0);
+                    signs = __builtin_amdgcn_alignbit(signs, __float_as_uint(d0), 31);
+                    signs = __builtin_amdgcn_alignbit(signs, __float_as_uint(d), 31);
+                    if (i == 0) asm("v_min_f32 %0, |%1|, |%2|" : "=v"(near) : "v"(d0), "v"(d));
+                    else asm("v_min3_f32 %0, %0, |%1|, |%2|" : "+v"(near) : "v"(d0), "v"(d));
+                }
+                const bool risky = ROLLOFF_EXACT_ALL || (cum_total != 0.0f && (!(near > cum_total * ROLL_GUARD) || cum_total < 1e-30f));
+                int expo = 0, zero = 0;
+                double mant = 1.0;
+#pragma unroll
+                for (int h = 0; h < 2; h++) {
+                    const float c7 = h == 1 ? m15 : cur.m[7];
+                    const float* c8 = cur.m + 8 * h;
+                    double g = ((double)c8[0] * (double)c8[1]) * ((double)c8[2] * (double)c8[3]);
+                    g *= 3.273390607896142e150;
+                    g *= ((double)c8[4] * (double)c8[5]) * ((double)c8[6] * (double)c7);
+                    if (g == 0.0) zero = 1;
+                    const uint64_t bits = (uint64_t)__double_as_longlong(g);
+                    expo += (int)(bits >> 52);
+                    mant *= __longlong_as_double((long long)((bits & 0xFFFFFFFFFFFFFull) | 0x3FF0000000000000ull));
+                }
+                const int red = row16_sum((int)((uint32_t)__popc(signs) | ((uint32_t)zero << 9) | ((uint32_t)expo << 14)));
+                const int c = red & 511, any_zero = (red >> 9) & 31, exps = (int)((uint32_t)red >> 14);
+                mant = row16_prod(mant);
+                const bool mine = l == (r & 15);
+                const uint64_t risky_lanes = __builtin_amdgcn_ballot_w64(risky);
+                const uint32_t grp_mask = (uint32_t)(risky_lanes >> (threadIdx.x & 48)) & 0xFFFFu;
+                const int packed = c | (any_zero ? 1 << 9 : 0) | (cum_total == 0.0f ? 1 << 10 : 0) | (exps << 11) | (grp_mask != 0 ? 1 << 27 : 0);
+                st_total = mine ? total : st_total;
+                st_wtotal = mine ? wtotal : st_wtotal;
+                st_ints = mine ? packed : st_ints;
+                st_mant = mine ? (float)mant : st_mant;
+                if (risky_lanes != 0) {
+                    if (grp_mask != 0) {
+                        float4* dst = reinterpret_cast<float4*>(fix->mags + (size_t)(sd.t_off + (uint64_t)(k_begin + r)) * 256 + 16 * l);
+                        dst[0] = make_float4(cur.m[0], cur.m[1], cur.m[2], cur.m[3]);
+                        dst[1] = make_float4(cur.m[4], cur.m[5], cur.m[6], cur.m[7]);
+                        dst[2] = make_float4(cur.m[8], cur.m[9], cur.m[10], cur.m[11]);
+                        dst[3] = make_float4(cur.m[12], cur.m[13], cur.m[14], m15);
+                    }
+                }
+            }
+        };
+        auto finish16 = [&](int r16) {
+            const int r = r16 + l;
+            const long k = k_begin + r;
+            if (r < len && r < lim_t) {
+                const float cbin = (st_total == 0.0f) ? 0.0f : st_wtotal / st_total;
+                const int st_c = st_ints & 511, st_exps = (st_ints >> 11) & 0xFFFF;
+                const float rbin = (st_ints & (1 << 10)) ? 0.0f : (float)((st_c < 256) ? st_c + 1 : 256);
+                float flat = 0.0f;
+                if (!(st_ints & (1 << 9))) {
+                    const float geo = exp2f((log2f(st_mant) + (float)st_exps) / 256.0f - (1023.0f + 500.0f) / 8.0f);
+                    if (geo != 0.0f) flat = geo / (st_total / 256.0f);
+                }
+                centroid[sd.t_off + k] = freq_per_bin * fmaxf(cbin, 0.0f);
+                rolloff[sd.t_off + k] = (st_ints & (1 << 27)) ? ROLLOFF_UNPROVEN : freq_per_bin * fmaxf(rbin, 0.0f);
+                flatness[sd.t_off + k] = flat;
+            }
+        };
+
+        for (int rb = 0; rb < len; rb += 4) {
+            frame(std::integral_constant<int, 0>{}, rb, B, A);
+            __builtin_amdgcn_sched_barrier(0);
+            if (rb + 1 < len) frame(std::integral_constant<int, 1>{}, rb + 1, B, A);
+            __builtin_amdgcn_sched_barrier(0);
+            if (rb + 2 < len) frame(std::integral_constant<int, 2>{}, rb + 2, A, B);
+            __builtin_amdgcn_sched_barrier(0);
+            if (rb + 3 < len) frame(std::integral_constant<int, 3>{}, rb + 3, A, B);
+            __builtin_amdgcn_sched_barrier(0);
+            if ((rb & 15) == 12 || rb + 4 >= len) finish16(rb & ~15);
+        }
+
+        __syncthreads();
+        if (grp + 1 < GROUPS_PER_WG && k_begin + FRAMES_PER_GROUP + 1 < (long)sd.n_f) {
+            const long q = (k_begin + FRAMES_PER_GROUP) >> 1;
             float f = 0.0f;
+            const float cn = halo[grp + 1][256];
             if constexpr (SEQ_FLUX) {
+            float hc[16];
+#pragma unroll
+            for (int e = 0; e < 16; e++) hc[e] = halo[grp + 1][16 * e + l];
 #pragma unroll 1
             for (int step = 0; step < 16; step++) {
                 const float carry = dpp_mov<0x111>(f);
                 if (l == step) {
                     f = carry;
 #pragma unroll
-                    for (int e = 0; e < 16; e++) f += fmaxf(cur.m[e] - prev.m[e], 0.0f);
-                }
-            }
-            f = __shfl(f, (threadIdx.x & 48) + 15, 64) + fmaxf(cur.nyq - prev.nyq, 0.0f);
-            ss = row16_sum(ss);
-            zc = (uint32_t)row16_sum((int)zc);
+                    for (int e = 0; e < 16; e++) f += fmaxf(hc[e] - A.m[e], 0.0f);
+                }
+            }
+            f = __shfl(f, (threadIdx.x & 48) + 15, 64) + fmaxf(cn - A.nyq, 0.0f);
             } else {
 #pragma unroll
-            for (int i = 0; i < 8; i++) {
-                const f2 d = mk(cur.m[2 * i], cur.m[2 * i + 1]) - mk(prev.m[2 * i], prev.m[2 * i + 1]);
-                f += fmaxf(d.x, 0.0f);
-                f += fmaxf(d.y, 0.0f);
-            }
-            if (l == 0) f += fmaxf(cur.nyq - prev.nyq, 0.0f);
-            row16_sum2f_1u(ss, f, zc);
-            }
-            if (l == 0) { e256[sd.e_off + q] = ss; zc256[sd.e_off + q] = zc; }
-            if (J == 1 && share && r == 1) {
-#pragma unroll
-                for (int e = 0; e < 16; e++) halo[grp][16 * e + l] = cur.m[e];
-                if (l == 0) halo[grp][256] = cur.nyq;
-            } else if (l == 0 && qr < lim_b) {
-                flux[sd.b_off + q] = f;
-            }
-        }
-        if (r < lim_t) {
-            const float m15 = (l == 15) ? cur.nyq : cur.m[15];
-            f2 s2 = mk(0.0f, 0.0f), e2 = mk(0.0f, 0.0f), q2 = mk(0.0f, 0.0f);
-#pragma unroll
-            for (int i = 0; i < 8; i++) {
-                const f2 mp = mk(cur.m[2 * i], i == 7 ? m15 : cur.m[2 * i + 1]);
-                s2 = s2 + mp;
-                e2 = e2 + mp * mk((float)(2 * i), (float)(2 * i + 1));
-                q2 = q2 + mp * mp;
-            }
-            auto hadd = [](f2 v) __attribute__((always_inline)) { float r; asm("v_add_f32 %0, %1, %2" : "=v"(r) : "v"(v.x), "v"(v.y)); return r; };
-            const float sum = hadd(s2), sqsum = hadd(q2);
-            const float wsum = (float)(16 * l) * sum + hadd(e2);
-            float total, wtotal, incl, cum_total;
-            row16_sum3_scan1(sum, wsum, sqsum, sqsum, total, wtotal, incl, cum_total);
-            const float thr = cum_total * 0.95f;
-            float d = (incl - sqsum) - thr;
-            float near;
-            uint32_t signs = 0;
-#pragma unroll
-            for (int i = 0; i < 8; i++) {
-                const float m0 = cur.m[2 * i], m1 = i == 7 ? m15 : cur.m[2 * i + 1];
-                const float d0 = fmaf(m0, m0, d);
-                d = fmaf(m1, m1, d0);
-                signs = __builtin_amdgcn_alignbit(signs, __float_as_uint(d0), 31);
-                signs = __builtin_amdgcn_alignbit(signs, __float_as_uint(d), 31);
-                if (i == 0) asm("v_min_f32 %0, |%1|, |%2|" : "=v"(near) : "v"(d0), "v"(d));
-                else asm("v_min3_f32 %0, %0, |%1|, |%2|" : "+v"(near) : "v"(d0), "v"(d));
-            }
-            const bool risky = ROLLOFF_EXACT_ALL || (cum_total != 0.0f && (!(near > cum_total * ROLL_GUARD) || cum_total < 1e-30f));
-            int expo = 0, zero = 0;
-            double mant = 1.0;
-#pragma unroll
-            for (int h = 0; h < 2; h++) {
-                const float c7 = h == 1 ? m15 : cur.m[7];
-                const float* c8 = cur.m + 8 * h;
-                double g = ((double)c8[0] * (double)c8[1]) * ((double)c8[2] * (double)c8[3]);
-                g *= 3.273390607896142e150;
-                g *= ((double)c8[4] * (double)c8[5]) * ((double)c8[6] * (double)c7);
-                if (g == 0.0) zero = 1;
-                const uint64_t bits = (uint64_t)__double_as_longlong(g);
-                expo += (int)(bits >> 52);
-                mant *= __longlong_as_double((long long)((bits & 0xFFFFFFFFFFFFFull) | 0x3FF0000000000000ull));
-            }
-            const int red = row16_sum((int)((uint32_t)__popc(signs) | ((uint32_t)zero << 9) | ((uint32_t)expo << 14)));
-            const int c = red & 511, any_zero = (red >> 9) & 31, exps = (int)((uint32_t)red >> 14);
-            mant = row16_prod(mant);
-            const bool mine = l == (r & 15);
-            const uint64_t risky_lanes = __builtin_amdgcn_ballot_w64(risky);
-            const uint32_t grp_mask = (uint32_t)(risky_lanes >> (threadIdx.x & 48)) & 0xFFFFu;
-            const int packed = c | (any_zero ? 1 << 9 : 0) | (cum_total == 0.0f ? 1 << 10 : 0) | (exps << 11) | (grp_mask != 0 ? 1 << 27 : 0);
-            st_total = mine ? total : st_total;
-            st_wtotal = mine ? wtotal : st_wtotal;
-            st_ints = mine ? packed : st_ints;
-            st_mant = mine ? (float)mant : st_mant;
-            if (risky_lanes != 0) {
-                if (grp_mask != 0) {
-                    float4* dst = reinterpret_cast<float4*>(fix->mags + (size_t)(sd.t_off + (uint64_t)(k_begin + r)) * 256 + 16 * l);
-                    dst[0] = make_float4(cur.m[0], cur.m[1], cur.m[2], cur.m[3]);
-                    dst[1] = make_float4(cur.m[4], cur.m[5], cur.m[6], cur.m[7]);
-                    dst[2] = make_float4(cur.m[8], cur.m[9], cur.m[10], cur.m[11]);
-                    dst[3] = make_float4(cur.m[12], cur.m[13], cur.m[14], m15);
-                }
-            }
-        }
-    };
-    auto finish16 = [&](int r16) {
-        const int r = r16 + l;
-        const long k = k_begin + r;
-        if (r < len && r < lim_t) {
-            const float cbin = (st_total == 0.0f) ? 0.0f : st_wtotal / st_total;
-            const int st_c = st_ints & 511, st_exps = (st_ints >> 11) & 0xFFFF;
-            const float rbin = (st_ints & (1 << 10)) ? 0.0f : (float)((st_c < 256) ? st_c + 1 : 256);
-            float flat = 0.0f;
-            if (!(st_ints & (1 << 9))) {
-                const float geo = exp2f((log2f(st_mant) + (float)st_exps) / 256.0f - (1023.0f + 500.0f) / 8.0f);
-                if (geo != 0.0f) flat = geo / (st_total / 256.0f);
-            }
-            centroid[sd.t_off + k] = freq_per_bin * fmaxf(cbin, 0.0f);
-            rolloff[sd.t_off + k] = (st_ints & (1 << 27)) ? ROLLOFF_UNPROVEN : freq_per_bin * fmaxf(rbin, 0.0f);
-            flatness[sd.t_off + k] = flat;
-        }
-    };
-
-    for (int rb = 0; rb < len; rb += 4) {
-        frame(std::integral_constant<int, 0>{}, rb, B, A);
-        __builtin_amdgcn_sched_barrier(0);
-        if (rb + 1 < len) frame(std::integral_constant<int, 1>{}, rb + 1, B, A);
-        __builtin_amdgcn_sched_barrier(0);
-        if (rb + 2 < len) frame(std::integral_constant<int, 2>{}, rb + 2, A, B);
-        __builtin_amdgcn_sched_barrier(0);
-        if (rb + 3 < len) frame(std::integral_constant<int, 3>{}, rb + 3, A, B);
-        __builtin_amdgcn_sched_barrier(0);
-        if ((rb & 15) == 12 || rb + 4 >= len) finish16(rb & ~15);
-    }
-
-    __syncthreads();
-    if (grp + 1 < GROUPS_PER_WG && k_begin + FRAMES_PER_GROUP + 1 < (long)sd.n_f) {
-        const long q = (k_begin + FRAMES_PER_GROUP) >> 1;
-        float f = 0.0f;
-        const float cn = halo[grp + 1][256];
-        if constexpr (SEQ_FLUX) {
-        float hc[16];
-#pragma unroll
-        for (int e = 0; e < 16; e++) hc[e] = halo[grp + 1][16 * e + l];
-#pragma unroll 1
-        for (int step = 0; step < 16; step++) {
-            const float carry = dpp_mov<0x111>(f);
-            if (l == step) {
-                f = carry;
-#pragma unroll
-                for (int e = 0; e < 16; e++) f += fmaxf(hc[e] - A.m[e], 0.0f);
-            }
-        }
-        f = __shfl(f, (threadIdx.x & 48) + 15, 64) + fmaxf(cn - A.nyq, 0.0f);
-        } else {
-#pragma unroll
-        for (int e = 0; e < 16; e++) {
-            const float c = halo[grp + 1][16 * e + l];
-            f += fmaxf(c - A.m[e], 0.0f);
-        }
-        if (l == 0) f += fmaxf(cn - A.nyq, 0.0f);
-        f = row16_sum(f);
-        }
-        if (l == 0 && q < (long)sd.n_b) flux[sd.b_off + q] = f;
-    }
-
-    if (active && k_end == (long)sd.n_f) {
-        const float* __restrict__ x = pcm + sd.pcm_off;
-        const uint64_t t0 = (uint64_t)sd.n_f * HOP_T;
-        for (uint64_t q = t0 >> 8; q < (uint64_t)sd.n_e; q++) {
-            const uint64_t lo = (q << 8) > t0 ? (q << 8) : t0;
-            const uint64_t hi = ((q + 1) << 8) < sd.n ? ((q + 1) << 8) : sd.n;
-            for (uint64_t i = lo + (uint64_t)l; i < hi; i += 16) {
-                const float v = x[i], pv = x[i - 1];
-                ss_acc += v * v;
-                zc_acc += ((v > 0.0f) != (pv > 0.0f)) ? 1u : 0u;
-            }
-            const float ss = row16_sum(ss_acc);
-            const uint32_t zc = (uint32_t)row16_sum((int)zc_acc);
-            if (l == 0) { e256[sd.e_off + q] = ss; zc256[sd.e_off + q] = zc; }
-            ss_acc = 0.0f;
-            zc_acc = 0;
-        }
-    }
-}
-
-void launch_fft512(const Batch& b, const Workspace& w, const DeviceTables& t, hipStream_t st, bool rolloff_exact_all, bool seq_flux) {
+            for (int e = 0; e < 16; e++) {
+                const float c = halo[grp + 1][16 * e + l];
+                f += fmaxf(c - A.m[e], 0.0f);
+            }
+            if (l == 0) f += fmaxf(cn - A.nyq, 0.0f);
+            f = row16_sum(f);
+            }
+            if (l == 0 && q < (long)sd.n_b) flux[sd.b_off + q] = f;
+        }
+
+        if (active && k_end == (long)sd.n_f) {
+            const float* __restrict__ x = pcm + sd.pcm_off;
+            const uint64_t t0 = (uint64_t)sd.n_f * HOP_T;
+            for (uint64_t q = t0 >> 8; q < (uint64_t)sd.n_e; q++) {
+                const uint64_t lo = (q << 8) > t0 ? (q << 8) : t0;
+                const uint64_t hi = ((q + 1) << 8) < sd.n ? ((q + 1) << 8) : sd.n;
+                for (uint64_t i = lo + (uint64_t)l; i < hi; i += 16) {
+                    const float v = x[i], pv = x[i - 1];
+                    ss_acc += v * v;
+                    zc_acc += ((v > 0.0f) != (pv > 0.0f)) ? 1u : 0u;
+                }
+                const float ss = row16_sum(ss_acc);
+                const uint32_t zc = (uint32_t)row16_sum((int)zc_acc);
+                if (l == 0) { e256[sd.e_off + q] = ss; zc256[sd.e_off + q] = zc; }
+                ss_acc = 0.0f;
+                zc_acc = 0;
+            }
+        }
+    }
+}
+
+void launch_fft512(const Batch& b, const Workspace& w, const DeviceTables& t, hipStream_t st, uint32_t resident_wgs, bool rolloff_exact_all, bool seq_flux) {
     if (b.tiles_f == 0) return;
     auto k = fft512_kernel<false, false>;
     if (rolloff_exact_all && seq_flux) k = fft512_kernel<true, true>;
     else if (rolloff_exact_all) k = fft512_kernel<true, false>;
     else if (seq_flux) k = fft512_kernel<false, true>;
-    hipLaunchKernelGGL(k, dim3(b.tiles_f), dim3(256), 0, st, b.pcm, b.songs, b.n_songs, b.pfx_f, t.hannz512,
-                       t.tw512, w.centroid, w.rolloff, w.flatness, w.flux, w.e256, w.zc256, w.roll_fix);
-}
-
-}
+    const WalkPlan plan = walk_plan(b.tiles_f, F512_WALK_K, resident_wgs);
+    hipLaunchKernelGGL(k, dim3(walk_grid(plan)), dim3(256), 0, st, b.pcm, b.songs, b.n_songs, b.pfx_f, t.hannz512,
+                       t.tw512, w.centroid, w.rolloff, w.flatness, w.flux, w.e256, w.zc256, w.roll_fix, plan);
+}
+
+}
diff --git a/bliss-rs_amd/csrc/scheduler.hip b/bliss-rs_amd/csrc/scheduler.hip
--- a/bliss-rs_amd/csrc/scheduler.hip
+++ b/bliss-rs_amd/csrc/scheduler.hip
@@ -29,7 +29,7 @@
     size_t b = 0;
     b += (size_t)d.n_t * 12 + (size_t)d.n_b * 8 + (size_t)d.n_e * 8;
     b += (size_t)d.n_c * (CBINS_PAD * 4 + 4);
-    b += (size_t)H1_BINS * 4 + N_TUNING * 4 + sizeof(TuningState) + sizeof(TempoState);
+    b += (size_t)H1_BINS * 4 + (N_TUNING + 1) * 4 + sizeof(TuningState) + sizeof(TempoState);
     b += (size_t)d.n_c * CAND_BUDGET_PER_FRAME * 9;
     b += (size_t)d.n_c * (PIP_MAX_PER_FRAME * 4 + 4);
     b += ((size_t)d.n_c / CH_TILE + 1) * 80;
@@ -70,7 +70,8 @@
     w.roll_fix_bytes = (size_t)(reinterpret_cast<uint8_t*>(w.peak_rec + t.tot_c * PIP_MAX_PER_FRAME) - reinterpret_cast<uint8_t*>(w.spec));
     w.frame_max = m.take<float>(t.tot_c);
     w.roll_fix = m.take<RollFix>(1);
-    w.h1 = m.take<uint32_t>((size_t)ns * H1_BINS); w.hist100 = m.take<uint32_t>((size_t)ns * N_TUNING);
+    w.h1 = m.take<uint32_t>((size_t)ns * H1_BINS); w.hist100 = m.take<uint32_t>((size_t)ns * (N_TUNING + 1));
+    w.tune_tickets = w.hist100 + (size_t)ns * N_TUNING;
     w.tuning = m.take<TuningState>(ns);
     w.peak_cnt = m.take<uint32_t>(t.tot_c);
     w.cand_mag = m.take<double>(t.cand_cap); w.cand_pb = m.take<uint8_t>(t.cand_cap);
@@ -186,9 +187,9 @@
     HIP_TRY(hipEventRecord(slot.ev_desc, st));
 
     HIP_TRY(hipMemsetAsync(w.h1, 0, (size_t)ns * H1_BINS * 4, st));
-    HIP_TRY(hipMemsetAsync(w.hist100, 0, (size_t)ns * N_TUNING * 4, st));
+    HIP_TRY(hipMemsetAsync(w.hist100, 0, (size_t)ns * (N_TUNING + 1) * 4, st));
     HIP_TRY(hipMemsetAsync(w.cand_cursor, 0, 16, st));
-    { Prof p(c, K_FFT512); launch_fft512(b, w, c->tables, st, c->rolloff_exact_all, c->flux_order); }
+    { Prof p(c, K_FFT512); launch_fft512(b, w, c->tables, st, 2u * (uint32_t)c->n_cus, c->rolloff_exact_all, c->flux_order); }
     { Prof p(c, K_ROLLFIX); launch_rolloff_fix(b, w, t.tot_t, st); }
     if (multi) {
         HIP_TRY(hipEventRecord(slot.ev_fork, st));
@@ -238,7 +239,6 @@
                 if (acf_early) launch_beat_track(b, w, c->tables, sb); else launch_beat(b, w, c->tables, sb);
             }
             { Prof p(c, K_TUNE_PASS2, sc); launch_tune_pass2(b, w, sc, &slot.piece[k]); }
-            { Prof p(c, K_TUNE_FINAL, sc); launch_tune_final(b, w, sc, &slot.piece[k]); }
             HIP_TRY(hipEventRecord(slot.ev_piece[k], sc));
         }
         if (beat_last) {
@@ -260,7 +260,6 @@
         if (acf_early) launch_beat_track(b, w, c->tables, sb); else launch_beat(b, w, c->tables, sb);
     }
     { Prof p(c, K_TUNE_PASS2, sc); launch_tune_pass2(b, w, sc); }
-    { Prof p(c, K_TUNE_FINAL, sc); launch_tune_final(b, w, sc); }
     if (multi) HIP_TRY(hipEventRecord(slot.ev_tune, sc));
     if (beat_last) {
         HIP_TRY(hipStreamWaitEvent(sb, slot.ev_tune, 0));
diff --git a/bliss-rs_amd/csrc/tile_walk.hpp b/bliss-rs_amd/csrc/tile_walk.hpp
--- /dev/null
+++ b/bliss-rs_amd/csrc/tile_walk.hpp
@@ -0,0 +1,71 @@
+#pragma once
+#include <stdint.h>
+
+#if defined(__HIPCC__)
+#define BG_WALK_FN __host__ __device__ __forceinline__
+#else
+#define BG_WALK_FN inline
+#endif
+
+namespace bg {
+
+#ifndef F512_WALK_K
+#define F512_WALK_K 8
+#endif
+
+constexpr int WALK_MAX_PHASES = 4;
+struct WalkPlan {
+    uint32_t n_phases;
+    uint32_t block0[WALK_MAX_PHASES + 1];
+    uint32_t tile0[WALK_MAX_PHASES + 1];
+};
+
+BG_WALK_FN WalkPlan walk_plan(uint32_t tiles, uint32_t k, uint32_t resident) {
+    WalkPlan p{};
+    if (resident == 0) resident = 1;
+    uint32_t len[WALK_MAX_PHASES], cnt[WALK_MAX_PHASES];
+    uint32_t n = 0, left = tiles;
+    if (k == 0) {
+        len[0] = 0; cnt[0] = tiles; n = 1; left = 0;
+    } else {
+        for (uint32_t kk = 1; kk < k && n + 1 < (uint32_t)WALK_MAX_PHASES && left > 0; kk *= 2) {
+            const uint64_t want = (uint64_t)resident * kk;
+            len[n] = kk; cnt[n] = want < left ? (uint32_t)want : left;
+            left -= cnt[n]; n++;
+        }
+        if (left > 0 || n == 0) { len[n] = k; cnt[n] = left; left = 0; n++; }
+    }
+    uint32_t b = 0, t = 0;
+    for (uint32_t i = 0; i < n; i++) {
+        const uint32_t q = n - 1 - i;
+        if (cnt[q] == 0) continue;
+        p.block0[p.n_phases] = b; p.tile0[p.n_phases] = t; p.n_phases++;
+        b += len[q] == 0 ? (cnt[q] < resident ? cnt[q] : resident) : (uint32_t)(((uint64_t)cnt[q] + len[q] - 1) / len[q]);
+        t += cnt[q];
+    }
+    p.block0[p.n_phases] = b; p.tile0[p.n_phases] = t;
+    return p;
+}
+BG_WALK_FN uint32_t walk_grid(const WalkPlan& p) { return p.block0[p.n_phases]; }
+
+BG_WALK_FN void walk_enter(const WalkPlan& p, uint32_t b, uint32_t* first, uint32_t* stride, uint32_t* end) {
+    *first = *end = 0; *stride = 1;
+    for (uint32_t ph = 0; ph < p.n_phases; ph++)
+        if (b >= p.block0[ph] && b < p.block0[ph + 1]) {
+            *stride = p.block0[ph + 1] - p.block0[ph];
+            *first = p.tile0[ph] + (b - p.block0[ph]);
+            *end = p.tile0[ph + 1];
+        }
+}
+
+BG_WALK_FN uint32_t walk_locate(const uint32_t* __restrict__ prefix, uint32_t n_songs, uint32_t tile, uint32_t* tile_in_song) {
+    uint32_t lo = 0, hi = n_songs;
+    while (hi - lo > 1) {
+        const uint32_t mid = (lo + hi) >> 1;
+        if (prefix[mid] <= tile) lo = mid; else hi = mid;
+    }
+    *tile_in_song = tile - prefix[lo];
+    return lo;
+}
+
+}
```

Measured after the change: 22810 songs/sec. -18.1%, worse.
